# icrdr/3D-UNet-Renal-Anatomy-Extraction

Measured on AMD Instinct MI355X. Metric: train voxels/sec (128^3 patch, bs=2 per GPU), whole job, higher is better.
Workload: dtype bf16; 1 GPU; ResUnet3D(num_pool=4, num_features=32, in=1, out=3) train step (fwd+HybirdLoss+bwd+Adam), 2x1x128^3 per GPU, dropout on; global_batch=2, parallelism=dp1, optimizer=optim.Adam (fused multi-tensor)

## Files before the change

### 3d-unet-renal-anatomy-extraction_amd/_native.py

```python
import ctypes
import os
import threading

import torch

_HERE = os.path.dirname(os.path.abspath(__file__))
LIB_PATH = os.environ.get("RU3D_LIB", os.path.join(_HERE, "libru3d.so"))

F32, BF16, F16 = 0, 1, 2
PREDICT_MAX_BATCH = 16
LABEL_I64, LABEL_U8 = 0, 1
ROLE_CONV_FWD, ROLE_CONV_DGRAD, ROLE_CONVT_FWD, ROLE_CONVT_DGRAD, ROLE_BIAS = 0, 1, 2, 3, 4
LOSS_HYBIRD, LOSS_DICELOSS, LOSS_FOCAL, LOSS_DICE = 0, 1, 2, 3
MAX_CLASSES = 8


class Tensor(ctypes.Structure):
    _fields_ = [("ptr", ctypes.c_void_p), ("n", ctypes.c_int32), ("d", ctypes.c_int32), ("h", ctypes.c_int32),
                ("w", ctypes.c_int32), ("c", ctypes.c_int32), ("ld", ctypes.c_int32), ("cseg", ctypes.c_int32),
                ("seg_stride", ctypes.c_int64)]


class PackItem(ctypes.Structure):
    _fields_ = [("src", ctypes.c_void_p), ("dst", ctypes.c_void_p), ("cout", ctypes.c_int32), ("cin", ctypes.c_int32),
# ... 31 lines not shown
                ("y0", ctypes.c_int32), ("w", ctypes.c_int32), ("h", ctypes.c_int32), ("X", ctypes.c_int32),
                ("Y", ctypes.c_int32), ("Z", ctypes.c_int32), ("C", ctypes.c_int32), ("channel", ctypes.c_int32),
                ("kind", ctypes.c_int32), ("axis", ctypes.c_int32), ("index", ctypes.c_int32),
                ("overlay_mode", ctypes.c_int32 * 2)]


class RenderView(ctypes.Structure):
    _fields_ = [("o", ctypes.c_double * 3), ("du", ctypes.c_double * 3), ("dv", ctypes.c_double * 3),
                ("dw", ctypes.c_double * 3), ("spacing", ctypes.c_double * 3), ("light", ctypes.c_double * 3),
                ("ambient", ctypes.c_double), ("diffuse", ctypes.c_double), ("background", ctypes.c_double * 3),
                ("num_steps", ctypes.c_int32), ("reserved", ctypes.c_int32)]


class DsLevel(ctypes.Structure):
    _fields_ = [("logits", ctypes.c_void_p), ("stride_n", ctypes.c_int64), ("stride_c", ctypes.c_int64),
                ("stride_v", ctypes.c_int64), ("d", ctypes.c_int32), ("h", ctypes.c_int32), ("w", ctypes.c_int32),
                ("shift", ctypes.c_int32)]


DS_MAX_LEVELS = 8
MASK_NE, MASK_EQ, MASK_GT, MASK_GE = 0, 1, 2, 3
TILE_F32, TILE_U8 = 0, 1
OVERLAY_FILL, OVERLAY_OUTLINE = 0, 1
RENDER_MAX_TILES = 256
MORPH_ERODE, MORPH_DILATE = 0, 1
MORPH_MAX_EXTENT, MORPH_MAX_ROWS = 15, 225
CONFUSION_MAX_CLASSES = 32
ORDER_STATS_MAX_RANKS = 8
EDT_MAX_AXIS = 4096
SPATIAL_MAX_YZ = 2560
BOUNDARY_MAX_AXIS = 2048
DEGRADE_MAX_RADIUS = 16
PACK_MAX = 40
_P = ctypes.POINTER(Tensor)
_vp, _i, _i64, _f, _sz, _u64 = (ctypes.c_void_p, ctypes.c_int, ctypes.c_int64, ctypes.c_float, ctypes.c_size_t,
                                ctypes.c_uint64)
_dbl = ctypes.c_double

SIGNATURES = {
    "ru3d_version": (_i, []),
    "ru3d_last_error": (ctypes.c_char_p, []),
    "ru3d_launch_log_begin": (None, []),
    "ru3d_launch_log_end": (ctypes.c_char_p, []),
    "ru3d_packed_weight_bytes": (_sz, [_i, _i, _i, _i, _i, _i]),
    "ru3d_pack_weight": (_i, [_vp, _vp, _i, _i, _i, _i, _i, _i, _vp]),
    "ru3d_pack_weights": (_i, [ctypes.POINTER(PackItem), _i, _i, _vp]),
    "ru3d_unpad_weight_grad": (_i, [_vp, _vp, _i, _i, _i, _i, _i, _vp]),
    "ru3d_conv3d_workspace_bytes": (_sz, [_P, _P, _i, _i, _i]),
    "ru3d_conv3d_fwd": (_i, [_P, _vp, _vp, _P, _P, _i, _i, _i, _i, _vp, _sz, _vp]),
    "ru3d_conv3d_fwd_in_workspace_bytes": (_sz, [_P, _P, _i, _i, _i]),
    "ru3d_conv3d_fwd_in": (_i, [_P, _vp, _vp, _P, _i, _i, _i, _vp, _vp, _vp, _vp, _sz, _f, _vp]),
    "ru3d_conv3d_fwd_in_lrelu_workspace_bytes": (_sz, [_P, _P, _i, _i, _i]),
    "ru3d_conv3d_fwd_in_lrelu": (_i, [_P, _vp, _vp, _P, _i, _i, _i, _vp, _vp, _vp, _P, _P, _f, _vp, _sz, _f, _vp]),
    "ru3d_planar_concat_supported": (_i, [_i, _i, _i, _i, _i, _i, _i]),
    "ru3d_conv3d_dgrad": (_i, [_P, _vp, _P, _P, _i, _i, _i, _vp, _sz, _vp]),
    "ru3d_conv3d_s2_pair_fwd_in_supported": (_i, [_P, _P, _P, _i]),
    "ru3d_conv3d_s2_pair_fwd_in_workspace_bytes": (_sz, [_P, _P, _i]),
    "ru3d_conv3d_s2_pair_fwd_in": (_i, [_P, _vp, _vp, _P, _vp, _vp, _P, _vp, _vp, _vp, _vp, _sz, _f, _i, _vp]),
    "ru3d_conv3d_s1_dgrad_pair_supported": (_i, [_P, _P, _P, _i]),
    "ru3d_conv3d_s1_dgrad_pair": (_i, [_P, _vp, _P, _vp, _P, _i, _vp]),
    "ru3d_conv3d_s2_dgrad_pair_supported": (_i, [_P, _P, _P, _P, _i]),
    "ru3d_conv3d_s2_dgrad_pair": (_i, [_P, _vp, _P, _vp, _P, _P, _i, _vp]),
    "ru3d_conv3d_wgrad_workspace_bytes": (_sz, [_P, _P, _i, _i, _i]),
    "ru3d_conv3d_wgrad": (_i, [_P, _P, _vp, _vp, _sz, _i, _i, _i, _vp]),
    "ru3d_conv3d_wgrad_bias_workspace_bytes": (_sz, [_P, _P, _i, _i, _i]),
    "ru3d_conv3d_wgrad_bias": (_i, [_P, _P, _vp, _vp, _vp, _sz, _i, _i, _i, _vp]),
    "ru3d_conv3d_wgrad_pair_supported": (_i, [_P, _P, _P, _i, _i]),
    "ru3d_conv3d_wgrad_pair_workspace_bytes": (_sz, [_P, _P, _P, _i, _i]),
    "ru3d_conv3d_wgrad_pair": (_i, [_P, _P, _P, _vp, _vp, _vp, _sz, _i, _i, _vp]),
    "ru3d_head_bwd_supported": (_i, [_P, _P, _P, _i]),
    "ru3d_head_bwd_workspace_bytes": (_sz, [_P, _i]),
    "ru3d_head_bwd": (_i, [_P, _P, _vp, _i, _P, _vp, _vp, _vp, _sz, _i, _vp]),
    "ru3d_convtranspose3d_k3s2p1_fwd": (_i, [_P, _vp, _vp, _P, _i, _vp]),
    "ru3d_convtranspose3d_k3s2p1_fwd_in_workspace_bytes": (_sz, [_P, _P, _i]),
    "ru3d_convtranspose3d_k3s2p1_fwd_in": (_i, [_P, _vp, _vp, _P, _vp, _vp, _vp, _sz, _f, _i, _vp]),
    "ru3d_convtranspose3d_k3s2p1_dgrad": (_i, [_P, _vp, _P, _i, _vp]),
    "ru3d_convtranspose3d_k3s2p1_wgrad_workspace_bytes": (_sz, [_P, _P, _i]),
    "ru3d_convtranspose3d_k3s2p1_wgrad": (_i, [_P, _P, _vp, _vp, _sz, _i, _vp]),
    "ru3d_reduce_workspace_bytes": (_sz, [_P]),
    "ru3d_instnorm_stats": (_i, [_P, _vp, _vp, _vp, _vp, _sz, _f, _i, _vp]),
    "ru3d_in_lrelu_fwd": (_i, [_P, _vp, _vp, _P, _P, _f, _i, _vp]),
    "ru3d_skip1x1_in_lrelu_fwd_supported": (_i, [_P, _P, _P, _i]),
    "ru3d_skip1x1_in_lrelu_fwd": (_i, [_P, _vp, _vp, _P, _vp, _vp, _P, _f, _i, _vp]),
    "ru3d_in_lrelu_bwd": (_i, [_P, _P, _P, _vp, _vp, _P, _P, _vp, _sz, _f, _i, _vp, _vp, _i, _vp]),
    "ru3d_in_lrelu_bwd_apply": (_i, [_P, _P, _vp, _vp, _vp, _P, _f, _i, _i, _vp]),
    "ru3d_conv3d_dgrad_in_bwd_workspace_bytes": (_sz, [_P, _P, _i, _i, _i]),
    "ru3d_conv3d_dgrad_in_bwd": (_i, [_P, _vp, _P, _vp, _vp, _P, _P, _i, _i, _f, _i, _vp, _sz, _vp]),
    "ru3d_channel_sum": (_i, [_P, _vp, _vp, _sz, _i, _vp]),
    "ru3d_batchnorm_stats_pool": (_i, [_P, _vp, _vp, _vp, _sz, _i, _vp]),
    "ru3d_batchnorm_stats_finalize": (_i, [_vp, _i, _i, _i, _dbl, _vp, _vp, _vp, _f, _f, _vp, _vp, _vp, _vp, _vp, _vp, _vp]),
    "ru3d_affine_lrelu_fwd": (_i, [_P, _vp, _vp, _P, _P, _f, _i, _vp]),
    "ru3d_batchnorm_bwd_pool": (_i, [_P, _P, _P, _vp, _vp, _P, _vp, _vp, _sz, _f, _i, _vp]),
    "ru3d_batchnorm_bwd_apply": (_i, [_P, _P, _vp, _vp, _vp, _vp, _dbl, _P, _vp, _sz, _i, _i, _vp]),
    "ru3d_dropout3d_scale": (_i, [_vp, _i, _f, _u64, _u64, _vp]),
    "ru3d_dropout3d_scale_dev": (_i, [_vp, _i, _f, _u64, _u64, _vp, _vp]),
    "ru3d_pointwise": (_i, [_i, _P, _P, _P, _P, _P, _f, _i, _vp]),
    "ru3d_copy_channels": (_i, [_P, _P, _i, _vp]),
    "ru3d_add": (_i, [_P, _P, _P, _i, _vp]),
    "ru3d_cast_f32": (_i, [_P, _P, _i, _vp]),
    "ru3d_ncdhw_to_ndhwc": (_i, [_vp, _P, _i, _vp]),
    "ru3d_ndhwc_to_ncdhw": (_i, [_P, _vp, _i, _vp]),
    "ru3d_loss_state_bytes": (_sz, [_i]),
    "ru3d_loss_state_bad_labels_offset": (_sz, []),
    "ru3d_loss_workspace_bytes": (_sz, [_i, _i64, _i]),
    "ru3d_loss_fwd": (_i, [_vp, _i64, _i64, _i64, _vp, _i, _i, _i64, _i, _i, _f, _vp, _f, _f, _f, _vp, _vp, _vp,
                           _sz, _vp]),
    "ru3d_loss_bwd": (_i, [_vp, _i64, _i64, _i64, _vp, _i, _i, _i64, _i, _f, _vp, _vp, _vp, _i, _vp]),
    "ru3d_tversky": (_i, [_vp, _vp, _i64, _f, _f, _f, _vp, _vp, _sz, _vp]),
    "ru3d_predict_accumulate": (_i, [_P, _i, _i, _vp, _vp, _i, _i, _i, _i, _i, _i, _vp]),
    "ru3d_predict_merge": (_i, [_vp, _vp, _i, _i, _i, _i, _i, _i, _i, _i, _i, _i, _i, _vp, _vp]),
    "ru3d_predict_gather": (_i, [_vp, _i, _i, _i, _i, _vp, _i, _P, _vp]),
    "ru3d_predict_accumulate_weighted": (_i, [_P, _i, _i, _i, _vp, _vp, _vp, _vp, _vp, _i, _i, _i, _i, _i, _i, _vp]),
    "ru3d_components_workspace_bytes": (_sz, [_i, _i, _i]),
    "ru3d_label_components": (_i, [_vp, _i, _i, _i, _vp, _vp, _vp, _sz, _vp]),
    "ru3d_component_stats": (_i, [_vp, _i, _i, _i, _i, _vp, _vp, _vp]),
    "ru3d_filter_components_workspace_bytes": (_sz, [_i]),
    "ru3d_filter_components": (_i, [_vp, _i, _i, _i, _i, _vp, _i, _vp, _vp, _vp, _vp, _sz, _vp]),
    "ru3d_region_accumulate": (_i, [_vp, _i, _i, _i, _i, _i, _i, _i, _vp, _vp, _i, _i, _i, _vp]),
    "ru3d_cascade_merge": (_i, [_vp, _vp, _i, _i, _i, _i, _vp, _vp]),
    "ru3d_mask_bytes": (_sz, [_i, _i, _i]),
    "ru3d_mask_pack": (_i, [_vp, _i, _i, _i, _i, _i, _vp, _vp]),
    "ru3d_mask_unpack": (_i, [_vp, _i, _i, _i, _i, _i, _vp, _vp]),
    "ru3d_binary_morph": (_i, [_vp, _vp, _i, _i, _i, _i, ctypes.POINTER(MorphRow), _i, _i, _vp]),
    "ru3d_confusion_counts": (_i, [_vp, _vp, _i64, _i, _vp, _vp]),
    "ru3d_threshold_bbox": (_i, [_vp, _i, _i, _i, _i, _f, _vp, _vp, _vp]),
    "ru3d_masked_sample_workspace_bytes": (_sz, [_i, _i, _i]),
    "ru3d_masked_sample": (_i, [_vp, _i, _i, _i, _i, _i, _vp, _i, _i, _vp, _i64, _vp, _vp, _sz, _vp]),
    "ru3d_order_stats_workspace_bytes": (_sz, []),
    "ru3d_order_stats": (_i, [_vp, _i64, ctypes.POINTER(ctypes.c_int64), _i, _vp, _vp, _sz, _vp]),
    "ru3d_moments_workspace_bytes": (_sz, []),
    "ru3d_moments": (_i, [_vp, _i64, _vp, _vp, _sz, _vp]),
    "ru3d_edt_workspace_bytes": (_sz, [_i, _i, _i]),
    "ru3d_edt_squared": (_i, [_vp, _i, _i, _i, ctypes.POINTER(_dbl), _vp, _vp, _sz, _vp]),
    "ru3d_mask_surface": (_i, [_vp, _vp, _i, _i, _i, _vp]),
    "ru3d_edt_gather_workspace_bytes": (_sz, [_i, _i, _i]),
    "ru3d_edt_gather": (_i, [_vp, _vp, _i, _i, _i, _vp, _i64, _vp, _vp, _sz, _vp]),
    "ru3d_edt_reduce_workspace_bytes": (_sz, [_i64]),
    "ru3d_edt_reduce": (_i, [_vp, _vp, _i64, _dbl, _vp, _vp, _sz, _vp]),
    "ru3d_skeleton_workspace_bytes": (_sz, [_i, _i, _i]),
    "ru3d_skeleton_thin": (_i, [_vp, _i, _i, _i, _i, _vp, _sz, _vp]),
    "ru3d_skeleton_classify": (_i, [_vp, _i, _i, _i, _vp, _vp, _vp, _vp]),
    "ru3d_skeleton_length": (_i, [_vp, _i, _i, _i, ctypes.POINTER(_dbl), _vp, _vp, _sz, _vp]),
    "ru3d_skeleton_overlap": (_i, [_vp, _vp, _i, _i, _i, _vp, _vp]),
    "ru3d_skeleton_radius_stats": (_i, [_vp, _i64, _vp, _vp]),
    "ru3d_cldice_workspace_bytes": (_sz, [_i, _i, _i, _i, _i]),
    "ru3d_cldice_state_bytes": (_sz, []),
    "ru3d_soft_skeleton_fwd": (_i, [_vp, _i, _i, _i, _i, _i, _vp, _vp, _vp, _vp, _vp, _sz, _vp]),
    "ru3d_soft_skeleton_bwd": (_i, [_vp, _i, _i, _i, _i, _i, _vp, _vp, _vp, _vp, _vp, _vp, _sz, _vp]),
    "ru3d_cldice_fwd": (_i, [_vp, _i64, _i64, _i64, _vp, _i, _i, _i, _i, _i, _i, _vp, _i, _i, _vp, _f, _vp, _vp, _vp,
                             _vp, _vp, _vp, _vp, _vp, _sz, _vp]),
    "ru3d_cldice_bwd": (_i, [_vp, _i64, _i64, _i64, _vp, _i, _i, _i, _i, _i, _i, _vp, _i, _i, _vp, _vp, _vp, _vp, _vp,
                             _vp, _vp, _f, _i, _vp, _vp, _sz, _vp]),
    "ru3d_boundary_workspace_bytes": (_sz, [_i, _i, _i, _i]),
    "ru3d_boundary_state_bytes": (_sz, []),
    "ru3d_signed_distance": (_i, [_vp, _i, _i, _i, _i, _i, _i, _vp, _i, _vp, _vp, _vp, _sz, _vp]),
    "ru3d_boundary_fwd": (_i, [_vp, _i64, _i64, _i64, _vp, _i, _i, _i, _i, _i, _i, _vp, _i, _vp, _vp, _vp, _vp, _vp,
                               _sz, _vp]),
    "ru3d_boundary_bwd": (_i, [_vp, _i64, _i64, _i64, _i, _i, _i, _i, _i, _vp, _i, _vp, _vp, _vp, _f, _i, _vp, _vp]),
    "ru3d_ds_state_bytes": (_sz, []),
    "ru3d_ds_state_bad_labels_offset": (_sz, []),
    "ru3d_ds_block_bytes": (_sz, []),
    "ru3d_ds_loss_workspace_bytes": (_sz, [ctypes.POINTER(DsLevel), _i, _i]),
    "ru3d_ds_loss_fwd": (_i, [ctypes.POINTER(DsLevel), _i, _vp, _i, _i, _i, _i, _i, _i, _i, _f, _vp, _f, _f, _f, _vp, _vp,
                              _vp, _vp, _sz, _vp]),
    "ru3d_ds_loss_bwd": (_i, [ctypes.POINTER(DsLevel), ctypes.POINTER(_vp), _i, _vp, _i, _i, _i, _i, _i, _i, _f, _vp, _vp,
                              _vp]),
# ... 217 lines not shown
```

### 3d-unet-renal-anatomy-extraction_amd/_ops.py

```python
import ctypes
import os
import threading
import weakref

import torch

import _native as N
from _native import check, desc, ptr, ref, stream

LRELU_SLOPE = 0.01
IN_EPS = 1e-5


def pack_weight(w, role, dtype, stride=1):
    N.require_device(w, "weight")
    w = w.detach()
    if w.dtype != torch.float32 or not w.is_contiguous():
        w = w.float().contiguous()
    k = w.shape[2]
    if role in (N.ROLE_CONVT_FWD, N.ROLE_CONVT_DGRAD):
        cin, cout = w.shape[0], w.shape[1]
    else:
        cout, cin = w.shape[0], w.shape[1]
    code = N.dtype_code(dtype)
# ... 431 lines not shown
        return None
    dx = N.new_act(2 * n, cin // 2, d, h, w, dy.dtype, dy.device) if planar else N.new_act(n, cin, d, h, w, dy.dtype, dy.device)
    ddy, ddy2, ddx = desc(dy), desc(dy2), desc(N.Split(dx) if planar else dx)
    if not N.lib.ru3d_conv3d_s1_dgrad_pair_supported(ref(ddy), ref(ddy2), ref(ddx), code):
        return None
    check(N.lib.ru3d_conv3d_s1_dgrad_pair(ref(ddy), ptr(pw3), ref(ddy2), ptr(pw1), ref(ddx), code, stream()),
          "conv3d_s1_dgrad_pair")
    return dx


def conv_s2_dgrad_pair(dy, pw3, dy2, pw1, in_shape, res=None):
    n, cin, d, h, w = in_shape
    code = N.dtype_code(dy.dtype)
    if code == N.F32:
        return None
    dx = N.new_act(n, cin, d, h, w, dy.dtype, dy.device)
    ddy, ddy2, ddx = desc(dy), desc(dy2), desc(dx)
    dr = desc(res) if res is not None else None
    if not N.lib.ru3d_conv3d_s2_dgrad_pair_supported(ref(ddy), ref(ddy2), ref(dr), ref(ddx), code):
        return None
    check(N.lib.ru3d_conv3d_s2_dgrad_pair(ref(ddy), ptr(pw3), ref(ddy2), ptr(pw1), ref(dr), ref(ddx), code, stream()),
          "conv3d_s2_dgrad_pair")
    return dx


def convt_dgrad(dy, pw, in_shape):
    n, cin, d, h, w = in_shape
    dx = N.new_act(n, cin, d, h, w, dy.dtype, dy.device)
    ddy, ddx = desc(dy), desc(dx)
    check(N.lib.ru3d_convtranspose3d_k3s2p1_dgrad(ref(ddy), ptr(pw), ref(ddx), N.dtype_code(dy.dtype), stream()),
          "convtranspose3d_dgrad")
    return dx


def convt_wgrad(x, dy, key=None):
    cin, cout = x.shape[1], dy.shape[1]
    dw = _grad_out(key, (cin, cout, 3, 3, 3), x.device)
    dx, ddy = desc(x), desc(dy)
    code = N.dtype_code(x.dtype)
    nbytes = N.lib.ru3d_convtranspose3d_k3s2p1_wgrad_workspace_bytes(ref(dx), ref(ddy), code)
    ws = N.workspace(nbytes, x.device)
    check(N.lib.ru3d_convtranspose3d_k3s2p1_wgrad(ref(dx), ref(ddy), ptr(dw), ptr(ws), ws.numel(), code, stream()),
          "convtranspose3d_wgrad")
    return dw


def in_stats(y, drop_scale=None):
    n, c = y.shape[0], y.shape[1]
    mean = torch.empty(n * c, dtype=torch.float32, device=y.device)
    scale = torch.empty(n * c, dtype=torch.float32, device=y.device)
    dy = desc(y)
    ws = N.workspace(N.lib.ru3d_reduce_workspace_bytes(ref(dy)), y.device)
    check(N.lib.ru3d_instnorm_stats(ref(dy), ptr(drop_scale), ptr(mean), ptr(scale), ptr(ws), ws.numel(), IN_EPS,
                                    N.dtype_code(y.dtype), stream()), "instnorm_stats")
    return mean, scale


def in_lrelu_fwd(y, mean, scale, res=None, out=None):
    if out is None:
        n, c, d, h, w = y.shape
        out = N.new_act(n, c, d, h, w, y.dtype, y.device)
    dy, do = desc(y), desc(out)
    dr = desc(res) if res is not None else None
    check(N.lib.ru3d_in_lrelu_fwd(ref(dy), ptr(mean), ptr(scale), ref(dr), ref(do), LRELU_SLOPE,
                                  N.dtype_code(y.dtype), stream()), "in_lrelu_fwd")
    return out


def skip1x1_in_lrelu_fwd(x, pw, bias, y, mean, scale, out=None):
    code = N.dtype_code(y.dtype)
    if code == N.F32:
        return None
    if out is None:
        n, c, d, h, w = y.shape
        out = N.new_act(n, c, d, h, w, y.dtype, y.device)
    dx, dy, do = desc(x), desc(y), desc(out)
    if not N.lib.ru3d_skip1x1_in_lrelu_fwd_supported(ref(dx), ref(dy), ref(do), code):
        return None
    check(N.lib.ru3d_skip1x1_in_lrelu_fwd(ref(dx), ptr(pw), ptr(_bias(bias)), ref(dy), ptr(mean), ptr(scale), ref(do),
                                          LRELU_SLOPE, code, stream()), "skip1x1_in_lrelu_fwd")
    return out


def in_lrelu_bwd(gout, out, y, mean, scale, want_gpre=False, zero_far=False, want_gpre_sum=False, dy_sum=None):
    n, c, d, h, w = y.shape
    dy = N.new_act(n, c, d, h, w, y.dtype, y.device)
    gpre = N.new_act(n, c, d, h, w, y.dtype, y.device) if want_gpre else None
    dg, do, dyy, ddy = desc(gout), desc(out), desc(y), desc(dy)
    dp = desc(gpre) if want_gpre else None
    ws = N.workspace(N.lib.ru3d_reduce_workspace_bytes(ref(dyy)), y.device)
    gsum = torch.empty(c, dtype=torch.float32, device=y.device) if (want_gpre and want_gpre_sum) else None
    check(N.lib.ru3d_in_lrelu_bwd(ref(dg), ref(do), ref(dyy), ptr(mean), ptr(scale), ref(ddy), ref(dp), ptr(ws),
                                  ws.numel(), LRELU_SLOPE, 1 if zero_far else 0, ptr(gsum), ptr(dy_sum),
                                  N.dtype_code(y.dtype), stream()), "in_lrelu_bwd")
    if want_gpre_sum:
        return dy, gpre, gsum
    return dy, gpre


_BN_SYNC = [None, 1]


def set_bn_sync(group=None, enable=True):
    import torch.distributed as dist
    if enable and dist.is_available() and dist.is_initialized() and dist.get_world_size(group) > 1:
        _BN_SYNC[0], _BN_SYNC[1] = (group if group is not None else dist.group.WORLD), dist.get_world_size(group)
    else:
        _BN_SYNC[0], _BN_SYNC[1] = None, 1


def _bn_allreduce(pooled):
    if _BN_SYNC[0] is not None:
        import torch.distributed as dist
        dist.all_reduce(pooled, group=_BN_SYNC[0])
    return pooled


def bn_train_stats(y, drop_scale, norm, c_real):
    n, c = y.shape[0], y.shape[1]
    dev = y.device
    dy = desc(y)
    pooled = torch.empty(2 * c, dtype=torch.float64, device=dev)
    ws = N.workspace(N.lib.ru3d_reduce_workspace_bytes(ref(dy)), dev)
    check(N.lib.ru3d_batchnorm_stats_pool(ref(dy), ptr(drop_scale), ptr(pooled), ptr(ws), ws.numel(),
                                          N.dtype_code(y.dtype), stream()), "batchnorm_stats_pool")
    _bn_allreduce(pooled)
    count = float(n * y.shape[2] * y.shape[3] * y.shape[4]) * _BN_SYNC[1]
    track = norm.track_running_stats and norm.running_mean is not None
    momentum = 0.0
    if track:
        norm.num_batches_tracked.add_(1)
        momentum = (1.0 / float(norm.num_batches_tracked)) if norm.momentum is None else float(norm.momentum)
    out = torch.empty(4, n * c, dtype=torch.float32, device=dev)
    gamma = norm.weight.detach() if norm.weight is not None else None
    beta = norm.bias.detach() if norm.bias is not None else None
    for t in (gamma, beta, norm.running_mean if track else None, norm.running_var if track else None):
        if t is not None and (t.dtype != torch.float32 or not t.is_contiguous() or t.device != dev):
            raise N.Ru3dError("BatchNorm3d: parameters / running statistics must be contiguous fp32 on %s" % dev)
    check(N.lib.ru3d_batchnorm_stats_finalize(ptr(pooled), n, c, c_real, count, ptr(drop_scale), ptr(gamma), ptr(beta),
                                              float(norm.eps), momentum, ptr(norm.running_mean if track else None),
                                              ptr(norm.running_var if track else None), ptr(out[0]), ptr(out[1]),
                                              ptr(out[2]), ptr(out[3]), stream()), "batchnorm_stats_finalize")
    return out[0], out[1], out[2], out[3], count


def affine_lrelu_fwd(y, scale, shift, res=None, out=None):
    if out is None:
        n, c, d, h, w = y.shape
        out = N.new_act(n, c, d, h, w, y.dtype, y.device)
    dy, do = desc(y), desc(out)
    dr = desc(res) if res is not None else None
    check(N.lib.ru3d_affine_lrelu_fwd(ref(dy), ptr(scale), ptr(shift), ref(dr), ref(do), LRELU_SLOPE,
                                      N.dtype_code(y.dtype), stream()), "affine_lrelu_fwd")
    return out


def bn_lrelu_bwd(gout, out, y, a, b, fscale, count, zero_far=False):
    n, c, d, h, w = y.shape
    dev = y.device
    dy = N.new_act(n, c, d, h, w, y.dtype, dev)
    gpre = N.new_act(n, c, d, h, w, y.dtype, dev)
    dg, do, dyy, ddy, dp = desc(gout), desc(out), desc(y), desc(dy), desc(gpre)
    pooled = torch.empty(2 * c, dtype=torch.float64, device=dev)
    ws = N.workspace(N.lib.ru3d_reduce_workspace_bytes(ref(dyy)), dev)
    code = N.dtype_code(y.dtype)
    check(N.lib.ru3d_batchnorm_bwd_pool(ref(dg), ref(do), ref(dyy), ptr(a), ptr(b), ref(dp), ptr(pooled), ptr(ws),
# ... 215 lines not shown
    def skip_view(self, n, c, d, h, w, dtype, device):
        self.planar = False
        self.buf = N.new_act(n, self.up_channels + c, d, h, w, dtype, device)
        return self.buf[:, self.up_channels:]

    def planar_view(self, n, c, d, h, w, dtype, device):
        if (c != self.up_channels or dtype == torch.float32 or not self.dec_channels
                or not N.lib.ru3d_planar_concat_supported(n, d, h, w, c, self.dec_channels, N.dtype_code(dtype))):
            return None
        self.planar = True
        self.buf = N.new_act(2 * n, c, d, h, w, dtype, device)
        return self.buf[n:]


def _f32_view(pack, count):
    return pack[:4 * count].view(torch.float32)


class ConvFn(torch.autograd.Function):

    @staticmethod
    def forward(ctx, x, weight, bias, stride, storage_dtype, out_dtype, pad_in=False, pad_out=False):
        xin = as_input(x, storage_dtype)
        k = weight.shape[2]
        cout, cin = weight.shape[0], weight.shape[1]
        cin_seg = seg_of(cin, xin.shape[1]) if pad_in else 0
        cout_seg = cout if pad_out else 0
        if not pad_in and xin.shape[1] != cin:
            raise N.Ru3dError("conv: input has %d channels, weight expects %d" % (xin.shape[1], cin))
        cout_p = padded_dim(cout, cout_seg)
        specs = [(weight, N.ROLE_CONV_FWD, stride, cout_seg, cin_seg)]
        if ctx.needs_input_grad[0]:
            specs.append((weight, N.ROLE_CONV_DGRAD, stride, cout_seg, cin_seg))
        if cout_seg and bias is not None:
            specs.append((bias, N.ROLE_BIAS, 1, cout_seg, 0))
        packs = pack_weights(specs, storage_dtype)
        b = _f32_view(packs[-1], cout_p) if (cout_seg and bias is not None) else bias
        y = conv_fwd(xin, packs[0], b, cout_p, k, stride, out_dtype=out_dtype)
        ctx.save_for_backward(xin, packs[1] if ctx.needs_input_grad[0] else None)
        ctx.dims = (cout, cin, cout_seg, cin_seg)
        ctx.stride, ctx.k, ctx.has_bias = stride, k, bias is not None
        ctx.storage_dtype = storage_dtype
        ctx.in_dtype = x.dtype
        ctx.wkey = weight.data_ptr() if not (cout_seg or cin_seg) else None
        ctx.weight_ref = weight if (k == 1 and cout <= 4) else None
        return y

    @staticmethod
    def backward(ctx, gy):
        xin, pwd = ctx.saved_tensors
        sd = ctx.storage_dtype
        cout, cin, cout_seg, cin_seg = ctx.dims
        if (ctx.k == 1 and ctx.stride == 1 and cout <= 4 and not cout_seg and all(ctx.needs_input_grad[:2])
                and ctx.weight_ref is not None):
            fused = head_bwd(xin, gy, ctx.weight_ref, ctx.has_bias and ctx.needs_input_grad[2],
                             key=None if cin_seg else ctx.wkey)
            if fused is not None:
                gx, gw, gb = fused
                if gx.dtype != ctx.in_dtype:
                    gx = gx.to(ctx.in_dtype)
                return gx, gw, gb, None, None, None, None, None
        gy = as_grad(gy, sd)
        gx = gw = gb = None
        with _OnSide(gy.device):
            if ctx.needs_input_grad[1] and ctx.has_bias and ctx.needs_input_grad[2] and not (cout_seg or cin_seg) \
                    and sd != torch.float32:
                gw, gb = conv_wgrad_bias(xin, gy, ctx.k, ctx.stride, key=ctx.wkey)
            elif ctx.needs_input_grad[1]:
                gw = unpad_wgrad(conv_wgrad(xin, gy, ctx.k, ctx.stride, key=ctx.wkey), cout, cin, cout_seg, cin_seg)
            if gb is None and ctx.has_bias and ctx.needs_input_grad[2]:
                gb = channel_sum(gy)[:cout]
        if ctx.needs_input_grad[0]:
            gx = conv_dgrad(gy, pwd, tuple(xin.shape), ctx.k, ctx.stride)
            if gx.dtype != ctx.in_dtype:
                gx = gx.to(ctx.in_dtype)
        _join(gy.device, gw, gb)
        return gx, gw, gb, None, None, None, None, None


class ResBlockFn(torch.autograd.Function):

    @staticmethod
    def forward(ctx, x, w1, b1, w2, b2, ws, bs, stride, drop_scale, pad=0, checkpoint=False, in_link=None,
                out_link=None, planar=False):
        sd = x.dtype
        x = N.to_ndhwc(x)
        xt = x
        if planar:
            x = N.Split(x)
        cout, cin = w1.shape[0], w1.shape[1]
        cin_seg = seg_of(cin, x.shape[1], int(pad)) if pad else 0
        cout_seg = cout if pad else 0
        if not pad and x.shape[1] != cin:
            raise N.Ru3dError("ResBlock: input has %d channels, conv1 expects %d" % (x.shape[1], cin))
        cout_p = padded_dim(cout, cout_seg)
        train = any(ctx.needs_input_grad)
        need_gx = ctx.needs_input_grad[0]
        specs = [(w1, N.ROLE_CONV_FWD, stride, cout_seg, cin_seg), (w2, N.ROLE_CONV_FWD, 1, cout_seg, cout_seg)]
        if ws is not None:
            specs.append((ws, N.ROLE_CONV_FWD, stride, cout_seg, cin_seg))
        nfwd = len(specs)
        if train:
            specs.append((w2, N.ROLE_CONV_DGRAD, 1, cout_seg, cout_seg))
            if need_gx:
                specs.append((w1, N.ROLE_CONV_DGRAD, stride, cout_seg, cin_seg))
                if ws is not None:
                    specs.append((ws, N.ROLE_CONV_DGRAD, stride, cout_seg, cin_seg))
        nw = len(specs)
        if cout_seg:
            specs += [(b, N.ROLE_BIAS, 1, cout_seg, 0) for b in (b1, b2, bs) if b is not None]
        packs = pack_weights(specs, sd)
        if cout_seg:
            it = iter(packs[nw:])
            b1, b2, bs = [(_f32_view(next(it), cout_p) if b is not None else None) for b in (b1, b2, bs)]
        pw1, pw2 = packs[0], packs[1]
        fused = conv_s2_pair_fwd_in(x, pw1, b1, packs[2], bs, cout_p, drop_scale) if (ws is not None and stride == 2) else None
        if fused is not None:
            y1, mean1, scale1, skip = fused
            a1 = in_lrelu_fwd(y1, mean1, scale1)
        else:
            y1, mean1, scale1, a1 = conv_fwd_in_act(x, pw1, b1, cout_p, 3, stride, drop_scale)
        n_, _, d_, h_, w_ = a1.shape
        zout = None
        if out_link is not None and cout_p * a1.element_size() >= 128:
            zout = out_link.skip_view(n_, cout_p, d_, h_, w_, sd, x.device)
        elif out_link is not None:
            zout = out_link.planar_view(n_, cout_p, d_, h_, w_, sd, x.device)
        z = None
        tail = (fused is None and ws is not None and stride == 1 and out_link is None and sd != torch.float32
                and (x.shape[1], cout_p) in ((64, 32), (128, 64)) and n_ * d_ * h_ * w_ >= 65536)
        if tail:
            y2, mean2, scale2 = conv_fwd_in(a1, pw2, b2, cout_p, 3, 1)
            z = skip1x1_in_lrelu_fwd(x, packs[2], bs, y2, mean2, scale2)
            if z is None:
                z = in_lrelu_fwd(y2, mean2, scale2, res=conv_fwd(x, packs[2], bs, cout_p, 1, stride), out=zout)
        else:
            if fused is not None:
                pass
            elif ws is not None:
                skip = conv_fwd(x, packs[2], bs, cout_p, 1, stride)
            else:
                skip = x
            y2, mean2, scale2, z = conv_fwd_in_act(a1, pw2, b2, cout_p, 3, 1, res=skip, out=zout)
        bwd = packs[nfwd:nw] + [None] * 3
        if checkpoint and train:
            ctx.save_for_backward(xt, None, None, None, z, mean1, scale1, mean2, scale2, bwd[0], bwd[1], bwd[2],
                                  pw1, pw2, b1, b2)
        else:
            ctx.save_for_backward(xt, y1, a1, y2, z, mean1, scale1, mean2, scale2, bwd[0], bwd[1], bwd[2],
                                  None, None, None, None)
        ctx.planar = bool(planar)
        ctx.dims = (cout, cin, cout_seg, cin_seg)
        ctx.stride = stride
        plain = not (cout_seg or cin_seg)
        ctx.wkeys = (w1.data_ptr() if plain else None, w2.data_ptr() if plain else None,
                     ws.data_ptr() if (plain and ws is not None) else None)
        ctx.has_skip_conv = ws is not None
        ctx.in_link = in_link if (in_link is not None and ws is not None) else None
        if in_link is not None:
            in_link.fused_grad = ctx.in_link is not None and need_gx
        return z

    @staticmethod
    def backward(ctx, gz):
        (x, y1, a1, y2, z, mean1, scale1, mean2, scale2, pw2d, pw1d, pwsd, pw1, pw2, b1, b2) = ctx.saved_tensors
        cout, cin, cout_seg, cin_seg = ctx.dims
        cout_p = padded_dim(cout, cout_seg)
        sd = x.dtype
        dev = x.device
        stride = ctx.stride
        gz = as_grad(gz, sd)
        if ctx.planar:
            x = N.Split(x)
        if y1 is None:
            y1 = conv_fwd(x, pw1, b1, cout_p, 3, stride)
            a1 = in_lrelu_fwd(y1, mean1, scale1)
            y2 = conv_fwd(a1, pw2, b2, cout_p, 3, 1)
        dy2, gpre, gbs_sum = in_lrelu_bwd(gz, z, y2, mean2, scale2, want_gpre=True, want_gpre_sum=True)
        del y2
        return ResBlockFn._backward_tail(ctx, x, a1, y1, dy2, gpre, gbs_sum, mean1, scale1, pw2d, pw1d, pwsd)

    @staticmethod
    def _backward_tail(ctx, x, a1, y1, dy2, gpre, gbs_sum, mean1, scale1, pw2d, pw1d, pwsd):
        cout, cin, cout_seg, cin_seg = ctx.dims
        dev = x.device
        stride = ctx.stride
        gws = gbs = None
        nvox = dy2.shape[0] * dy2.shape[2] * dy2.shape[3] * dy2.shape[4]
        xk = x.t if ctx.planar else x
        pair_later = ctx.has_skip_conv and _wgrad_pair_ok(x, gpre, stride)
        with _OnSide(dev, nvox, (a1, dy2, xk, gpre)):
            gw2 = unpad_wgrad(conv_wgrad(a1, dy2, 3, 1, key=ctx.wkeys[1]), cout, cout, cout_seg, cout_seg)
            if ctx.has_skip_conv:
                if not pair_later:
                    gws = unpad_wgrad(conv_wgrad(x, gpre, 1, stride, key=ctx.wkeys[2]), cout, cin, cout_seg, cin_seg)
                gbs = gbs_sum[:cout]
        gb2 = None
        dy1 = conv_dgrad_in_bwd(dy2, pw2d, a1, mean1, scale1)
        del dy2, a1, y1
        with _OnSide(dev, nvox, (xk, dy1, gpre)):
            both = conv_wgrad_pair(x, dy1, gpre, stride, key=ctx.wkeys[0], key2=ctx.wkeys[2]) if pair_later else None
            if both is not None:
                gw1 = unpad_wgrad(both[0], cout, cin, cout_seg, cin_seg)
                gws = unpad_wgrad(both[1], cout, cin, cout_seg, cin_seg)
            else:
                gw1 = unpad_wgrad(conv_wgrad(x, dy1, 3, stride, key=ctx.wkeys[0]), cout, cin, cout_seg, cin_seg)
                if pair_later:
                    gws = unpad_wgrad(conv_wgrad(x, gpre, 1, stride, key=ctx.wkeys[2]), cout, cin, cout_seg, cin_seg)
        gb1 = None
        gx = None
        need_gx = ctx.needs_input_grad[0]
        if ctx.has_skip_conv:
            if need_gx:
                parked = None
                if ctx.in_link is not None:
                    parked, ctx.in_link.grad = ctx.in_link.grad, None
                if stride == 2:
                    gx = conv_s2_dgrad_pair(dy1, pw1d, gpre, pwsd, tuple(x.shape), res=parked)
                elif parked is None:
                    gx = conv_s1_dgrad_pair(dy1, pw1d, gpre, pwsd, tuple(x.shape), planar=ctx.planar)
                if gx is None and ctx.planar:
                    raise N.Ru3dError("ResBlock: the split concat input has no fused input-gradient kernel for this shape")
                if gx is None:
                    gx0 = conv_dgrad(gpre, pwsd, tuple(x.shape), 1, stride, res=parked)
                    gx = conv_dgrad(dy1, pw1d, tuple(x.shape), 3, stride, res=gx0)
        elif need_gx:
            gx = conv_dgrad(dy1, pw1d, tuple(x.shape), 3, stride, res=gpre)
        _join(dev, gw1, gw2, gws, gbs)
        return gx, gw1, gb1, gw2, gb2, gws, gbs, None, None, None, None, None, None, None


class UpFn(torch.autograd.Function):

    @staticmethod
    def forward(ctx, x, wt, bt, skip, pad=False, link=None):
        sd = x.dtype
        x = N.to_ndhwc(x)
        cin, cout = wt.shape[0], wt.shape[1]
        cin_seg = seg_of(cin, x.shape[1]) if pad else 0
        cout_seg = cout if pad else 0
        if not pad and x.shape[1] != cin:
            raise N.Ru3dError("ConvTrans3D: input has %d channels, weight expects %d" % (x.shape[1], cin))
        cout_p = padded_dim(cout, cout_seg)
        specs = [(wt, N.ROLE_CONVT_FWD, 2, cout_seg, cin_seg)]
        if ctx.needs_input_grad[0]:
            specs.append((wt, N.ROLE_CONVT_DGRAD, 2, cout_seg, cin_seg))
        if cout_seg and bt is not None:
            specs.append((bt, N.ROLE_BIAS, 1, cout_seg, 0))
        packs = pack_weights(specs, sd)
        btp = _f32_view(packs[-1], cout_p) if (cout_seg and bt is not None) else bt
        y, mean, scale = convt_fwd_in(x, packs[0], btp, cout_p)
        n, _, d, h, w = y.shape
        if skip is not None:
            skip = as_grad(skip, sd)
            cs = skip.shape[1]
            if tuple(skip.shape[2:]) != (d, h, w) or skip.shape[0] != n:
                raise N.Ru3dError("UpConcat: skip %s does not match up-sampled %s" % (tuple(skip.shape), tuple(y.shape)))
            planar = (link is not None and link.planar and link.buf is not None and link.up_channels == cout_p == cs
                      and tuple(link.buf.shape) == (2 * n, cs, d, h, w) and link.buf.dtype == sd
                      and skip.data_ptr() == link.buf[n:].data_ptr())
            in_place = (not planar and link is not None and not link.planar and link.buf is not None
                        and link.up_channels == cout_p
                        and tuple(link.buf.shape) == (n, cout_p + cs, d, h, w) and link.buf.dtype == sd
# ... 237 lines not shown
```

### 3d-unet-renal-anatomy-extraction_amd/csrc/api.hip

```cpp
#include "common.h"
#include "conv.h"
#include <string>

#ifndef RU3D_STORAGE_F16

static thread_local std::string g_last_error;

int ru3d_fail(int code, const char* fmt, ...) {
    char buf[512];
    va_list ap;
    va_start(ap, fmt);
    vsnprintf(buf, sizeof(buf), fmt, ap);
    va_end(ap);
    g_last_error = buf;
    return code;
}

static thread_local std::string g_launch_log;
static thread_local bool g_launch_log_armed = false;

int ru3d_check_launch(const char* what) {
    if (g_launch_log_armed) {
        if (!g_launch_log.empty()) g_launch_log += ';';
        g_launch_log += what;
// ... 331 lines not shown
    if (!mode || dtype != RU3D_BF16 || n <= 0 || d <= 0 || h <= 0 || w <= 0 || cseg != 32 || cout != 32) return 0;
    const int64_t V = (int64_t)d * h * w;
    if (((int64_t)n * V + V) * cseg * 2 >= (1ll << 31)) return 0;
    SlidePlan sp;
    if (!slide64_conv_plan(n, d, h, w, 2 * cseg, cout, &sp)) return 0;
    ConvGeom gd;
    gd.N = n; gd.Di = gd.Do = d; gd.Hi = gd.Ho = h; gd.Wi = gd.Wo = w; gd.Cin = cout; gd.Cout = 2 * cseg;
    gd.ldx = cout; gd.ldy = cseg; gd.CoutPad = 2 * cseg; gd.ldr = 0; gd.k = 3; gd.stride = 1; gd.pad = 1;
    gd.transposed = 0; gd.zero_far = 0; gd.flip = 1;
    static const int pair_mode = getenv("RU3D_DGRAD_PAIR") ? atoi(getenv("RU3D_DGRAD_PAIR")) : 1;
    if (!pair_mode || !mfma_conv_eligible(gd.Cin, gd.Cout, 3, dtype, dtype) || !mfma_conv_can_fuse_partner(gd)) return 0;
    WgradGeom gw;
    gw.N = n; gw.Di = gw.Do = d; gw.Hi = gw.Ho = h; gw.Wi = gw.Wo = w; gw.Cin = 2 * cseg; gw.Cout = cout;
    gw.ldx = cseg; gw.lddy = cout; gw.k = 3; gw.taps = 27; gw.stride = 1; gw.pad = 1;
    gw.s_o = (int64_t)gw.Cin * 27; gw.s_i = 27; gw.chunk_len = 0;
    WgradSlidePlan wp;
    if (!wgrad_slide_plan(gw, &wp)) return 0;
    static const int skip_mode = getenv("RU3D_FUSED_SKIP") ? atoi(getenv("RU3D_FUSED_SKIP")) : 1;
    if (!skip_mode || (V % 16) != 0 || V * n < 65536) return 0;
    return 1;
}

extern "C" int ru3d_conv3d_dgrad(const ru3d_tensor* dy, const void* w_packed, const ru3d_tensor* res,
                                 const ru3d_tensor* dx, int k, int stride, int dtype, void* ws, size_t ws_bytes,
                                 void* stream) {
    RU3D_FWD_F16(dtype, ru3d_conv3d_dgrad_f16(dy, w_packed, res, dx, k, stride, dtype, ws, ws_bytes, stream));
    Ru3dDeviceGuard dev_guard(stream);
    RU3D_REQUIRE(tensor_ok(dy) && tensor_ok(dx) && w_packed, "conv3d_dgrad: bad tensor/weight");
    RU3D_REQUIRE((k == 1 || k == 3) && (stride == 1 || stride == 2), "conv3d_dgrad: k=%d stride=%d unsupported", k, stride);
    RU3D_REQUIRE(dtype_ok(dtype), "conv3d_dgrad: bad dtype");
    RU3D_REQUIRE(dx->n == dy->n && dy->d == conv_out(dx->d, k, stride) && dy->h == conv_out(dx->h, k, stride) &&
                     dy->w == conv_out(dx->w, k, stride),
                 "conv3d_dgrad: dy extents (%d,%d,%d) do not match dx (%d,%d,%d) k=%d s=%d", dy->d, dy->h, dy->w,
                 dx->d, dx->h, dx->w, k, stride);
    RU3D_REQUIRE(res_ok(res, dx), "conv3d_dgrad: residual shape mismatch");
    if (stride == 1)
        return run_conv(dy, w_packed, nullptr, res, dx, k, 1, 0, 1, 0, dtype, dtype, as_stream(stream), ws, ws_bytes);
    return run_conv(dy, w_packed, nullptr, res, dx, k, stride, 1, 0, 0, dtype, dtype, as_stream(stream));
}

static ConvGeom dgrad_s1_geom(const ru3d_tensor* dy, const ru3d_tensor* da, int k);
extern "C" int ru3d_conv3d_s1_dgrad_pair_supported(const ru3d_tensor* dy, const ru3d_tensor* dy2, const ru3d_tensor* dx, int dtype) {
    RU3D_FWD_F16(dtype, ru3d_conv3d_s1_dgrad_pair_supported_f16(dy, dy2, dx, dtype));
    static const int mode = getenv("RU3D_DGRAD_PAIR") ? atoi(getenv("RU3D_DGRAD_PAIR")) : 1;
    if (!mode || dtype != RU3D_BF16 || !tensor_ok(dy) || !tensor_ok(dy2) || !tensor_ok_split(dx)) return 0;
    if (dx->cseg && (dx->cseg != 32 || dx->c != 64)) return 0;
    if (dy2->n != dy->n || dy2->d != dy->d || dy2->h != dy->h || dy2->w != dy->w || dy2->c != dy->c) return 0;
    if (dx->n != dy->n || dx->d != dy->d || dx->h != dy->h || dx->w != dy->w) return 0;
    if ((dy->ld % 8) || (dy2->ld % 8) || (dx->ld % 8)) return 0;
    if ((((uintptr_t)dy->ptr) | ((uintptr_t)dy2->ptr) | ((uintptr_t)dx->ptr)) % 16) return 0;
    if ((int64_t)dy->d * dy->h * dy->w * dy->ld >= (1ll << 30)) return 0;
    const ConvGeom g = dgrad_s1_geom(dy, dx, 3);
    return (mfma_conv_eligible(g.Cin, g.Cout, 3, dtype, dtype) && mfma_conv_can_fuse_partner(g)) ? 1 : 0;
}

extern "C" int ru3d_conv3d_s1_dgrad_pair(const ru3d_tensor* dy, const void* w3_packed, const ru3d_tensor* dy2,
                                         const void* w1_packed, const ru3d_tensor* dx, int dtype, void* stream) {
    RU3D_FWD_F16(dtype, ru3d_conv3d_s1_dgrad_pair_f16(dy, w3_packed, dy2, w1_packed, dx, dtype, stream));
    Ru3dDeviceGuard dev_guard(stream);
    RU3D_REQUIRE(w3_packed && w1_packed, "conv3d_s1_dgrad_pair: null weight");
    RU3D_REQUIRE(ru3d_conv3d_s1_dgrad_pair_supported(dy, dy2, dx, dtype),
                 "conv3d_s1_dgrad_pair: shapes have no fused kernel (ask ru3d_conv3d_s1_dgrad_pair_supported first)");
    const ConvGeom g = dgrad_s1_geom(dy, dx, 3);
    return conv_mfma_launch(dy->ptr, w3_packed, nullptr, nullptr, dx->ptr, g, as_stream(stream), nullptr, nullptr, 0, nullptr, 0,
                            0.f, dy2->ptr, dy2->ld, w1_packed);
}

extern "C" int ru3d_skip1x1_in_lrelu_fwd_supported(const ru3d_tensor* x, const ru3d_tensor* y, const ru3d_tensor* out, int dtype) {
    RU3D_FWD_F16(dtype, ru3d_skip1x1_in_lrelu_fwd_supported_f16(x, y, out, dtype));
    return skip1x1_fused_eligible(x, y, out, dtype) ? 1 : 0;
}

extern "C" int ru3d_skip1x1_in_lrelu_fwd(const ru3d_tensor* x, const void* w_packed, const float* bias, const ru3d_tensor* y,
                                         const float* mean, const float* scale, const ru3d_tensor* out, float slope, int dtype,
                                         void* stream) {
    RU3D_FWD_F16(dtype, ru3d_skip1x1_in_lrelu_fwd_f16(x, w_packed, bias, y, mean, scale, out, slope, dtype, stream));
    Ru3dDeviceGuard dev_guard(stream);
    RU3D_REQUIRE(w_packed && mean && scale, "skip1x1_in_lrelu_fwd: null argument");
    RU3D_REQUIRE(skip1x1_fused_eligible(x, y, out, dtype),
                 "skip1x1_in_lrelu_fwd: shapes have no fused kernel (ask ru3d_skip1x1_in_lrelu_fwd_supported first)");
    return skip1x1_fused_launch(x, w_packed, bias, y, mean, scale, out, slope, as_stream(stream));
}

extern "C" int ru3d_conv3d_s2_pair_fwd_in_supported(const ru3d_tensor* x, const ru3d_tensor* y3, const ru3d_tensor* y1, int dtype) {
    RU3D_FWD_F16(dtype, ru3d_conv3d_s2_pair_fwd_in_supported_f16(x, y3, y1, dtype));
    if (dtype != RU3D_BF16 || !tensor_ok(x) || !tensor_ok(y3) || !tensor_ok(y1)) return 0;
    if (y3->n != x->n || y3->d != conv_out(x->d, 3, 2) || y3->h != conv_out(x->h, 3, 2) || y3->w != conv_out(x->w, 3, 2)) return 0;
    if (y1->n != y3->n || y1->d != y3->d || y1->h != y3->h || y1->w != y3->w || y1->c != y3->c) return 0;
    if ((y1->ld % 4) || (int64_t)y1->d * y1->h * y1->w * y1->ld >= (1ll << 30)) return 0;
    if ((((uintptr_t)x->ptr) % 16) || ((((uintptr_t)y3->ptr) | ((uintptr_t)y1->ptr)) % 8)) return 0;
    return conv_s2_tile_eligible(fwd_geom(x, y3, 3, 2)) ? 1 : 0;
}

extern "C" size_t ru3d_conv3d_s2_pair_fwd_in_workspace_bytes(const ru3d_tensor* x, const ru3d_tensor* y3, int dtype) {
    RU3D_FWD_F16(dtype, ru3d_conv3d_s2_pair_fwd_in_workspace_bytes_f16(x, y3, dtype));
    if (!tensor_ok(x) || !tensor_ok(y3)) return 0;
    return conv_s2_tile_slab_bytes(fwd_geom(x, y3, 3, 2));
}

extern "C" int ru3d_conv3d_s2_pair_fwd_in(const ru3d_tensor* x, const void* w3_packed, const float* b3, const ru3d_tensor* y3,
                                          const void* w1_packed, const float* b1, const ru3d_tensor* y1,
                                          const float* drop_scale, float* mean, float* scale, void* ws, size_t ws_bytes,
                                          float eps, int dtype, void* stream) {
    RU3D_FWD_F16(dtype, ru3d_conv3d_s2_pair_fwd_in_f16(x, w3_packed, b3, y3, w1_packed, b1, y1, drop_scale, mean, scale, ws, ws_bytes, eps, dtype, stream));
    Ru3dDeviceGuard dev_guard(stream);
    RU3D_REQUIRE(w3_packed && w1_packed && mean && scale && ws, "conv3d_s2_pair_fwd_in: null argument");
    RU3D_REQUIRE(ru3d_conv3d_s2_pair_fwd_in_supported(x, y3, y1, dtype),
                 "conv3d_s2_pair_fwd_in: shapes have no fused kernel (ask ru3d_conv3d_s2_pair_fwd_in_supported first)");
    const ConvGeom g = fwd_geom(x, y3, 3, 2);
    const size_t slab = conv_s2_tile_slab_bytes(g);
    RU3D_REQUIRE(ws_bytes >= slab, "conv3d_s2_pair_fwd_in: workspace too small");
    int rc = conv_s2_tile_launch(x->ptr, w3_packed, b3, y3->ptr, g, (float*)ws, w1_packed, b1, y1->ptr, y1->ld, as_stream(stream));
    if (rc) return rc;
    int gx, cb;
    if (conv_s2_tile_slab_geom(g, &gx, &cb)) return ru3d_fail(-1, "conv3d_s2_pair_fwd_in: no slab geometry");
    return stats_slab_finalize_launch((const float*)ws, gx, cb, g.N, g.Cout, 1.0 / ((double)g.Do * g.Ho * g.Wo), drop_scale, eps,
                                      mean, scale, as_stream(stream));
}

static ConvGeom s2_dgrad_geom(const ru3d_tensor* dy, const ru3d_tensor* res, const ru3d_tensor* dx) {
    ConvGeom g;
    g.N = dy->n;
    g.Di = dy->d; g.Hi = dy->h; g.Wi = dy->w; g.Cin = dy->c; g.ldx = dy->ld;
    g.Do = dx->d; g.Ho = dx->h; g.Wo = dx->w; g.Cout = dx->c; g.ldy = dx->ld;
    g.CoutPad = generic_cout_pad(dx->c);
    g.ldr = res ? res->ld : 0;
    g.k = 3; g.stride = 2; g.pad = 1;
    g.transposed = 1; g.zero_far = 0; g.flip = 0;
    return g;
}

extern "C" int ru3d_conv3d_s2_dgrad_pair_supported(const ru3d_tensor* dy, const ru3d_tensor* dy2, const ru3d_tensor* res,
                                                   const ru3d_tensor* dx, int dtype) {
    RU3D_FWD_F16(dtype, ru3d_conv3d_s2_dgrad_pair_supported_f16(dy, dy2, res, dx, dtype));
    if (dtype != RU3D_BF16 || !tensor_ok(dy) || !tensor_ok(dy2) || !tensor_ok(dx) || !res_ok(res, dx)) return 0;
    if (dy2->n != dy->n || dy2->d != dy->d || dy2->h != dy->h || dy2->w != dy->w || dy2->c != dy->c) return 0;
    if (dx->n != dy->n || dy->d != conv_out(dx->d, 3, 2) || dy->h != conv_out(dx->h, 3, 2) || dy->w != conv_out(dx->w, 3, 2))
        return 0;
    if ((dy2->ld % 8) || (int64_t)dy2->d * dy2->h * dy2->w * dy2->ld >= (1ll << 30)) return 0;
    if ((((uintptr_t)dy->ptr) | ((uintptr_t)dy2->ptr) | ((uintptr_t)dx->ptr) | (res ? (uintptr_t)res->ptr : 0)) % 16) return 0;
    return convt_s2_tile_eligible(s2_dgrad_geom(dy, res, dx)) ? 1 : 0;
}

extern "C" int ru3d_conv3d_s2_dgrad_pair(const ru3d_tensor* dy, const void* w3_packed, const ru3d_tensor* dy2,
                                         const void* w1_packed, const ru3d_tensor* res, const ru3d_tensor* dx, int dtype,
                                         void* stream) {
    RU3D_FWD_F16(dtype, ru3d_conv3d_s2_dgrad_pair_f16(dy, w3_packed, dy2, w1_packed, res, dx, dtype, stream));
    Ru3dDeviceGuard dev_guard(stream);
    RU3D_REQUIRE(w3_packed && w1_packed, "conv3d_s2_dgrad_pair: null weight");
    RU3D_REQUIRE(ru3d_conv3d_s2_dgrad_pair_supported(dy, dy2, res, dx, dtype),
                 "conv3d_s2_dgrad_pair: shapes have no fused kernel (ask ru3d_conv3d_s2_dgrad_pair_supported first)");
    const ConvGeom g = s2_dgrad_geom(dy, res, dx);
    return convt_s2_tile_launch(dy->ptr, w3_packed, nullptr, res ? res->ptr : nullptr, dx->ptr, g, nullptr, dy2->ptr,
                                dy2->ld, w1_packed, as_stream(stream));
}

static ConvGeom dgrad_s1_geom(const ru3d_tensor* dy, const ru3d_tensor* da, int k) {
    ConvGeom g = fwd_geom(dy, da, k, 1);
    g.flip = 1;
    return g;
}

static bool dgrad_in_bwd_fused(const ru3d_tensor* dy, const ru3d_tensor* da, int k, int stride, int dtype) {
    static const int mode = getenv("RU3D_DGRAD_IN_FUSE") ? atoi(getenv("RU3D_DGRAD_IN_FUSE")) : 1;
    if (!mode || k != 3 || stride != 1 || dtype == RU3D_F32) return false;
    const ConvGeom g = dgrad_s1_geom(dy, da, k);
// ... 307 lines not shown
```

### 3d-unet-renal-anatomy-extraction_amd/csrc/conv.h

```cpp
#pragma once
#include "common.h"

namespace RU3D_NS {

struct ConvGeom {
    int N;
    int Di, Hi, Wi, Cin, ldx;
    int Do, Ho, Wo, Cout, ldy;
    int CoutPad;
    int ldr;
    int k, stride, pad;
    int transposed;
    int zero_far;
    int flip;
    int x_cseg = 0, y_cseg = 0;
    int64_t x_segstride = 0, y_segstride = 0;
};

struct WgradGeom {
    int N;
    int Di, Hi, Wi, Cin, ldx;
    int Do, Ho, Wo, Cout, lddy;
    int k, taps, stride, pad;
    int64_t s_o, s_i;
// ... 15 lines not shown
};
int pack_batch_launch(const PackBatch& b, int dtype, hipStream_t st);

struct PackPair {
    const float* src;
    void* dst_a;
    void* dst_b;
    int adim, bdim, taps;
    int a_real, a_pad, b_real, b_pad;
    int64_t s_a;
};
struct PackPairBatch {
    int count;
    PackPair item[RU3D_PACK_MAX];
};
int pack_pair_launch(const PackPairBatch& b, hipStream_t st);
int unpad_weight_launch(const float* src, float* dst, int cout, int cin, int taps, int co_real, int co_pad, int ci_real,
                        int ci_pad, int cin_p, hipStream_t st);

int generic_cot(int cout);
int generic_cout_pad(int cout);
int conv_generic_launch(const void* x, const void* w, const float* bias, const void* res, void* y,
                        const ConvGeom& g, int dtype, int y_dtype, hipStream_t st);
int pack_generic_launch(const float* src, void* dst, int cin, int cout, int taps, int64_t s_o, int64_t s_i,
                        int flip, int dtype, hipStream_t st);
size_t wgrad_generic_ws_bytes(const WgradGeom& g);
int wgrad_reduce_launch(const float* part, float* dw, int chunks, int taps, int cin, int cout, int64_t s_o, int64_t s_i,
                        hipStream_t st);
int wgrad_generic_launch(const void* x, const void* dy, float* dw, void* ws, size_t ws_bytes, WgradGeom g, int dtype,
                         hipStream_t st);

bool mfma_conv_eligible(int cin, int cout, int k, int dtype, int y_dtype);
bool mfma_conv_geometry_ok(const ConvGeom& g);
size_t mfma_packed_bytes(int cin, int cout, int taps);
int pack_mfma_launch(const float* src, void* dst, int cin, int cout, int taps, int64_t s_o, int64_t s_i, int flip,
                     hipStream_t st);
int conv_mfma_launch(const void* x, const void* w, const float* bias, const void* res, void* y, const ConvGeom& g,
                     hipStream_t st, float* stat_slab = nullptr, void* ws = nullptr, size_t ws_bytes = 0,
                     const void* bst_act = nullptr, int bst_ld = 0, float slope = 0.f, const void* x2 = nullptr,
                     int ldx2 = 0, const void* w2 = nullptr, int* defer_ks = nullptr);
bool mfma_conv_can_fuse_partner(const ConvGeom& g);
size_t conv_mfma_ws_bytes(const ConvGeom& g);
bool mfma_conv_can_fuse_stats(const ConvGeom& g);
size_t mfma_conv_stats_slab_bytes(const ConvGeom& g);
int mfma_conv_stats_finalize(const ConvGeom& g, const float* slab, const float* drop, float eps, float* mean,
                             float* scale, hipStream_t st);
int stats_slab_finalize_launch(const float* slab, int gx, int cb, int N, int C, double invV, const float* drop, float eps,
                               float* mean, float* scale, hipStream_t st);
bool mfma_conv_can_fuse_bwd_sums(const ConvGeom& g);
int mfma_conv_bwd_sums_finalize(const ConvGeom& g, const float* slab, float* m12, hipStream_t st);
bool mfma_wgrad_eligible(const WgradGeom& g, int dtype);
size_t wgrad_mfma_ws_bytes(const WgradGeom& g);
int wgrad_mfma_launch(const void* x, const void* dy, float* dw, void* ws, size_t ws_bytes, WgradGeom g,
                      hipStream_t st);

struct SlidePlan {
    int dsplit, DL, tiles_h, tiles_w, units, grid, ny;
};
bool slide_conv_plan(int N, int D, int H, int W, int Cin, int Cout, SlidePlan* out);
int conv_slide_launch(const void* x, const void* w, const float* bias, const void* res, void* y, const ConvGeom& g,
                      float* stat_slab, hipStream_t st, const void* bst_act = nullptr, int bst_ld = 0, float slope = 0.f,
                      const void* x2 = nullptr, int ldx2 = 0, const void* w2 = nullptr);

bool slide64_conv_plan(int N, int D, int H, int W, int Cin, int Cout, SlidePlan* out);
int conv_ws_slices(int N, int D, int H, int W, int Cin, int Cout);
int conv_ws_launch(const void* x, const void* w, float* part, int N, int D, int H, int W, int Cin, int Cout, int ldx,
                   int flip, int slices, hipStream_t st);
int conv_slide64_launch(const void* x, const void* w, const float* bias, const void* res, void* y, const ConvGeom& g,
                        float* stat_slab, hipStream_t st, const void* bst_act = nullptr, int bst_ld = 0, float slope = 0.f);

bool convt_s2_tile_eligible(const ConvGeom& g);
size_t convt_s2_tile_slab_bytes(const ConvGeom& g);
int convt_s2_tile_slab_geom(const ConvGeom& g, int* gx, int* cb);
int convt_s2_tile_launch(const void* x, const void* w, const float* bias, const void* res, void* y, const ConvGeom& g,
                         float* stat_slab, const void* x2, int ldx2, const void* w2, hipStream_t st);

bool conv_s2_tile_eligible(const ConvGeom& g);
size_t conv_s2_tile_slab_bytes(const ConvGeom& g);
int conv_s2_tile_slab_geom(const ConvGeom& g, int* gx, int* cb);
int conv_s2_tile_launch(const void* x, const void* w, const float* bias, void* y, const ConvGeom& g, float* stat_slab,
                        const void* w2, const float* bias2, void* y2, int ldy2, hipStream_t st);

bool skip1x1_fused_eligible(const ru3d_tensor* x, const ru3d_tensor* y2, const ru3d_tensor* out, int dtype);
int skip1x1_fused_launch(const ru3d_tensor* x, const void* w, const float* bias, const ru3d_tensor* y2, const float* mean,
                         const float* scale, const ru3d_tensor* out, float slope, hipStream_t st);

int in_small_mode(const ru3d_tensor* y, bool all_samples, const ru3d_tensor* a = nullptr, const ru3d_tensor* b = nullptr,
                  const ru3d_tensor* c = nullptr, const ru3d_tensor* d = nullptr);
size_t in_small_ws_bytes(const ru3d_tensor* y);
int in_small_fwd_launch(const ru3d_tensor* y, const float* part, int ksplit, const float* bias, const float* drop,
                        float* mean, float* scale, const ru3d_tensor* res, const ru3d_tensor* out, void* ws, float eps,
                        float slope, hipStream_t st);
int in_small_bwd_launch(const ru3d_tensor* gout, const float* part, int ksplit, const ru3d_tensor* outp,
                        const ru3d_tensor* y, const float* mean, const float* scale, const ru3d_tensor* dy,
                        const ru3d_tensor* gpre, void* ws, float slope, int zero_far, float* gpre_sum, hipStream_t st);

struct WgradSlidePlan {
    int dsplit, DL, tiles_h, tiles_w, units, G, pairs;
};
bool wgrad_slide_plan(const WgradGeom& g, WgradSlidePlan* out);
size_t wgrad_slide_ws_bytes(const WgradGeom& g);
int wgrad_slide_launch(const void* x, const void* dy, float* dw, void* ws, const WgradGeom& g, hipStream_t st);
size_t wgrad_slide_pair_ws_bytes(const WgradGeom& g);
int wgrad_slide_pair_launch(const void* x, const void* dy, const void* dy2, int lddy2, float* dw, float* dw2, void* ws,
                            const WgradGeom& g, hipStream_t st);

bool wgrad_s2_eligible(const WgradGeom& g);
size_t wgrad_s2_ws_bytes(const WgradGeom& g);
int wgrad_s2_launch(const void* x, const void* dy, float* dw, void* ws, const WgradGeom& g, hipStream_t st);
bool wgrad_s2_pair_eligible(const WgradGeom& g);
size_t wgrad_s2_pair_ws_bytes(const WgradGeom& g);
int wgrad_s2_pair_launch(const void* x, const void* dy, const void* dy2, int lddy2, float* dw, float* dw2, void* ws,
                         const WgradGeom& g, hipStream_t st);

bool stem_fwd_eligible(const ConvGeom& g, int dtype, int y_dtype, const void* res);
int stem_fwd_launch(const void* x, const void* w, const float* bias, void* y, const ConvGeom& g, int dtype,
                    hipStream_t st);
bool head_fwd_eligible(const ConvGeom& g, int dtype, const void* res);
int head_fwd_launch(const void* x, const void* w, const float* bias, void* y, const ConvGeom& g, int dtype,
                    int y_dtype, hipStream_t st);
bool head_dgrad_eligible(const ConvGeom& g, int dtype, int y_dtype, const void* res);
int head_dgrad_launch(const void* dy, const void* w, void* dx, const ConvGeom& g, int dtype, hipStream_t st);
bool stem_wgrad_eligible(const WgradGeom& g);
size_t stem_wgrad_ws_bytes(const WgradGeom& g);
int stem_wgrad_launch(const void* x, const void* dy, float* dw, void* ws, size_t ws_bytes, const WgradGeom& g,
                      int dtype, hipStream_t st, float* db = nullptr);
bool stem_wgrad_gives_bias(const WgradGeom& g, int dtype);
bool head_bwd_eligible(int Cin, int Cout, int dtype);
size_t head_bwd_ws_bytes(int64_t P, int Cin);
int head_bwd_launch(const void* a, int lda, const float* dlog, int ldd, const float* w, int cin_real, int Cin, int Cout,
                    void* dx, int lddx, float* dw, float* db, void* ws, int64_t P, hipStream_t st);
bool head_wgrad_eligible(const WgradGeom& g, int dtype);
size_t head_wgrad_ws_bytes(const WgradGeom& g);
int head_wgrad_launch(const void* x, const void* dy, float* dw, void* ws, size_t ws_bytes, const WgradGeom& g,
                      int dtype, hipStream_t st);

}
using namespace RU3D_NS;
```

### 3d-unet-renal-anatomy-extraction_amd/csrc/f16_names.h

```cpp
#pragma once
#define RU3D_F16_APIS(X) \
    X(ru3d_packed_weight_bytes) \
    X(ru3d_pack_weight) \
    X(ru3d_pack_weights) \
    X(ru3d_conv3d_workspace_bytes) \
    X(ru3d_conv3d_fwd) \
    X(ru3d_conv3d_fwd_in_workspace_bytes) \
    X(ru3d_conv3d_fwd_in) \
    X(ru3d_conv3d_fwd_in_lrelu) \
    X(ru3d_planar_concat_supported) \
    X(ru3d_conv3d_dgrad) \
    X(ru3d_conv3d_s2_pair_fwd_in_supported) \
    X(ru3d_conv3d_s2_pair_fwd_in_workspace_bytes) \
    X(ru3d_conv3d_s2_pair_fwd_in) \
    X(ru3d_conv3d_s1_dgrad_pair_supported) \
    X(ru3d_conv3d_s1_dgrad_pair) \
    X(ru3d_conv3d_s2_dgrad_pair_supported) \
    X(ru3d_conv3d_s2_dgrad_pair) \
    X(ru3d_convtranspose3d_k3s2p1_fwd_in_workspace_bytes) \
    X(ru3d_convtranspose3d_k3s2p1_fwd_in) \
    X(ru3d_conv3d_dgrad_in_bwd_workspace_bytes) \
    X(ru3d_conv3d_dgrad_in_bwd) \
    X(ru3d_in_lrelu_bwd_apply) \
    X(ru3d_conv3d_wgrad_workspace_bytes) \
    X(ru3d_conv3d_wgrad) \
    X(ru3d_conv3d_wgrad_bias_workspace_bytes) \
    X(ru3d_conv3d_wgrad_bias) \
    X(ru3d_conv3d_wgrad_pair_supported) \
    X(ru3d_conv3d_wgrad_pair_workspace_bytes) \
    X(ru3d_conv3d_wgrad_pair) \
    X(ru3d_head_bwd_supported) \
    X(ru3d_head_bwd_workspace_bytes) \
    X(ru3d_head_bwd) \
    X(ru3d_convtranspose3d_k3s2p1_fwd) \
    X(ru3d_convtranspose3d_k3s2p1_dgrad) \
    X(ru3d_convtranspose3d_k3s2p1_wgrad_workspace_bytes) \
    X(ru3d_convtranspose3d_k3s2p1_wgrad) \
    X(ru3d_instnorm_stats) \
    X(ru3d_in_lrelu_fwd) \
    X(ru3d_skip1x1_in_lrelu_fwd_supported) \
    X(ru3d_skip1x1_in_lrelu_fwd) \
    X(ru3d_in_lrelu_bwd) \
    X(ru3d_channel_sum) \
    X(ru3d_copy_channels) \
    X(ru3d_add) \
    X(ru3d_cast_f32) \
    X(ru3d_ncdhw_to_ndhwc) \
    X(ru3d_ndhwc_to_ncdhw) \
    X(ru3d_pointwise) \
    X(ru3d_batchnorm_stats_pool) \
    X(ru3d_affine_lrelu_fwd) \
    X(ru3d_batchnorm_bwd_pool) \
    X(ru3d_batchnorm_bwd_apply)

#ifdef RU3D_STORAGE_F16
#define ru3d_packed_weight_bytes ru3d_packed_weight_bytes_f16
#define ru3d_pack_weight ru3d_pack_weight_f16
#define ru3d_pack_weights ru3d_pack_weights_f16
#define ru3d_conv3d_workspace_bytes ru3d_conv3d_workspace_bytes_f16
#define ru3d_conv3d_fwd ru3d_conv3d_fwd_f16
#define ru3d_conv3d_fwd_in_workspace_bytes ru3d_conv3d_fwd_in_workspace_bytes_f16
#define ru3d_conv3d_fwd_in ru3d_conv3d_fwd_in_f16
#define ru3d_conv3d_fwd_in_lrelu ru3d_conv3d_fwd_in_lrelu_f16
#define ru3d_planar_concat_supported ru3d_planar_concat_supported_f16
#define ru3d_conv3d_dgrad ru3d_conv3d_dgrad_f16
#define ru3d_conv3d_s2_pair_fwd_in_supported ru3d_conv3d_s2_pair_fwd_in_supported_f16
#define ru3d_conv3d_s2_pair_fwd_in_workspace_bytes ru3d_conv3d_s2_pair_fwd_in_workspace_bytes_f16
#define ru3d_conv3d_s2_pair_fwd_in ru3d_conv3d_s2_pair_fwd_in_f16
#define ru3d_conv3d_s1_dgrad_pair_supported ru3d_conv3d_s1_dgrad_pair_supported_f16
#define ru3d_conv3d_s1_dgrad_pair ru3d_conv3d_s1_dgrad_pair_f16
#define ru3d_conv3d_s2_dgrad_pair_supported ru3d_conv3d_s2_dgrad_pair_supported_f16
#define ru3d_conv3d_s2_dgrad_pair ru3d_conv3d_s2_dgrad_pair_f16
#define ru3d_convtranspose3d_k3s2p1_fwd_in_workspace_bytes ru3d_convtranspose3d_k3s2p1_fwd_in_workspace_bytes_f16
#define ru3d_convtranspose3d_k3s2p1_fwd_in ru3d_convtranspose3d_k3s2p1_fwd_in_f16
#define ru3d_conv3d_dgrad_in_bwd_workspace_bytes ru3d_conv3d_dgrad_in_bwd_workspace_bytes_f16
#define ru3d_conv3d_dgrad_in_bwd ru3d_conv3d_dgrad_in_bwd_f16
#define ru3d_in_lrelu_bwd_apply ru3d_in_lrelu_bwd_apply_f16
#define ru3d_conv3d_wgrad_workspace_bytes ru3d_conv3d_wgrad_workspace_bytes_f16
#define ru3d_conv3d_wgrad ru3d_conv3d_wgrad_f16
#define ru3d_conv3d_wgrad_bias_workspace_bytes ru3d_conv3d_wgrad_bias_workspace_bytes_f16
#define ru3d_conv3d_wgrad_bias ru3d_conv3d_wgrad_bias_f16
#define ru3d_conv3d_wgrad_pair_supported ru3d_conv3d_wgrad_pair_supported_f16
#define ru3d_conv3d_wgrad_pair_workspace_bytes ru3d_conv3d_wgrad_pair_workspace_bytes_f16
#define ru3d_conv3d_wgrad_pair ru3d_conv3d_wgrad_pair_f16
#define ru3d_head_bwd_supported ru3d_head_bwd_supported_f16
#define ru3d_head_bwd_workspace_bytes ru3d_head_bwd_workspace_bytes_f16
#define ru3d_head_bwd ru3d_head_bwd_f16
#define ru3d_convtranspose3d_k3s2p1_fwd ru3d_convtranspose3d_k3s2p1_fwd_f16
#define ru3d_convtranspose3d_k3s2p1_dgrad ru3d_convtranspose3d_k3s2p1_dgrad_f16
#define ru3d_convtranspose3d_k3s2p1_wgrad_workspace_bytes ru3d_convtranspose3d_k3s2p1_wgrad_workspace_bytes_f16
#define ru3d_convtranspose3d_k3s2p1_wgrad ru3d_convtranspose3d_k3s2p1_wgrad_f16
#define ru3d_instnorm_stats ru3d_instnorm_stats_f16
#define ru3d_in_lrelu_fwd ru3d_in_lrelu_fwd_f16
#define ru3d_skip1x1_in_lrelu_fwd_supported ru3d_skip1x1_in_lrelu_fwd_supported_f16
#define ru3d_skip1x1_in_lrelu_fwd ru3d_skip1x1_in_lrelu_fwd_f16
#define ru3d_in_lrelu_bwd ru3d_in_lrelu_bwd_f16
#define ru3d_channel_sum ru3d_channel_sum_f16
#define ru3d_copy_channels ru3d_copy_channels_f16
#define ru3d_add ru3d_add_f16
#define ru3d_cast_f32 ru3d_cast_f32_f16
#define ru3d_ncdhw_to_ndhwc ru3d_ncdhw_to_ndhwc_f16
#define ru3d_ndhwc_to_ncdhw ru3d_ndhwc_to_ncdhw_f16
#define ru3d_pointwise ru3d_pointwise_f16
#define ru3d_batchnorm_stats_pool ru3d_batchnorm_stats_pool_f16
#define ru3d_affine_lrelu_fwd ru3d_affine_lrelu_fwd_f16
#define ru3d_batchnorm_bwd_pool ru3d_batchnorm_bwd_pool_f16
#define ru3d_batchnorm_bwd_apply ru3d_batchnorm_bwd_apply_f16
#endif
```

### 3d-unet-renal-anatomy-extraction_amd/csrc/fused_skip.hip

```cpp
#include "common.h"
#include "conv.h"

#include <type_traits>

namespace RU3D_NS {
namespace {

#ifdef RU3D_STORAGE_F16
#define RU3D_MFMA_16X16X32 __builtin_amdgcn_mfma_f32_16x16x32_f16
#else
#define RU3D_MFMA_16X16X32 __builtin_amdgcn_mfma_f32_16x16x32_bf16
#endif

template <int I, int N, typename F>
__device__ __forceinline__ void static_for(F&& f) {
    if constexpr (I < N) {
        f(std::integral_constant<int, I>{});
        static_for<I + 1, N>(f);
    }
}

typedef float f32x8 __attribute__((ext_vector_type(8)));

struct SkipArgs {
    const bf16* x;
    const bf16x8* w;
    const float* bias;
    const bf16* y2;
    const float* mean;
    const float* scale;
    bf16* out;
    int N;
    int64_t V;
    int ldx, ldy, ldo;
    int cout;
    float slope;
    int x_cseg;
    int64_t x_segstride;
};

template <int CIN, int NPB>
__global__ __launch_bounds__(256) void skip1x1_in_lrelu_fwd_kernel(SkipArgs a) {
    constexpr int KS = CIN / 32;
    const int lane = threadIdx.x & 63;
    const int p = lane & 15, g4 = lane >> 4;
    const int NTT = a.cout / 32;

    bf16x8 wreg[KS * NPB * 2];
    static_for<0, KS * NPB * 2>([&](auto ic) {
        constexpr int i = decltype(ic)::value;
        constexpr int ks = i / (NPB * 2), pb = (i / 2) % NPB, t = i & 1;
        const int co = pb * 32 + 8 * (p >> 2) + 4 * t + (p & 3);
        const int ci8 = ks * 4 + g4;
        wreg[i] = a.w[((ci8 >> 1) * NTT + (co >> 5)) * 64 + (co & 31) + 32 * (ci8 & 1)];
    });
    float bias8[NPB][8];
#pragma unroll
    for (int pb = 0; pb < NPB; pb++)
#pragma unroll
        for (int i = 0; i < 8; i++) bias8[pb][i] = a.bias ? a.bias[pb * 32 + 8 * g4 + i] : 0.f;

    const int64_t groups_per_sample = a.V / 16;
    const int64_t total = groups_per_sample * a.N;
    const int64_t wave_id = (int64_t)blockIdx.x * 4 + (threadIdx.x >> 6);
    const int64_t nwaves = (int64_t)gridDim.x * 4;
    int cur_n = -1;
    float mu[NPB][8], sc[NPB][8];
    for (int64_t gi = wave_id; gi < total; gi += nwaves) {
        const int n = (int)(gi / groups_per_sample);
        if (n != cur_n) {
            cur_n = n;
#pragma unroll
            for (int pb = 0; pb < NPB; pb++)
#pragma unroll
                for (int i = 0; i < 8; i++) {
                    mu[pb][i] = a.mean[n * a.cout + pb * 32 + 8 * g4 + i];
                    sc[pb][i] = a.scale[n * a.cout + pb * 32 + 8 * g4 + i];
                }
        }
        const int64_t vox = gi * 16 + p;
        bf16x8 xb[KS];
        static_for<0, KS>([&](auto kc) {
            constexpr int ks = decltype(kc)::value;
            const bf16* xp = a.x_cseg ? a.x + (int64_t)((ks * 32) / a.x_cseg) * a.x_segstride + (ks * 32) % a.x_cseg
                                      : a.x + ks * 32;
            xb[ks] = *reinterpret_cast<const bf16x8*>(xp + vox * a.ldx + g4 * 8);
        });
        bf16x8 yv[NPB];
#pragma unroll
        for (int pb = 0; pb < NPB; pb++) yv[pb] = *reinterpret_cast<const bf16x8*>(a.y2 + vox * a.ldy + pb * 32 + 8 * g4);
        f32x4 acc[NPB][2];
#pragma unroll
        for (int pb = 0; pb < NPB; pb++) {
            acc[pb][0] = f32x4{bias8[pb][0], bias8[pb][1], bias8[pb][2], bias8[pb][3]};
            acc[pb][1] = f32x4{bias8[pb][4], bias8[pb][5], bias8[pb][6], bias8[pb][7]};
        }
        static_for<0, KS>([&](auto kc) {
            constexpr int ks = decltype(kc)::value;
            static_for<0, NPB * 2>([&](auto tc) {
                constexpr int j = decltype(tc)::value;
                acc[j >> 1][j & 1] = RU3D_MFMA_16X16X32(wreg[ks * NPB * 2 + j], xb[ks], acc[j >> 1][j & 1], 0, 0, 0);
            });
        });
#pragma unroll
        for (int pb = 0; pb < NPB; pb++) {
            f32x4 a0 = acc[pb][0], a1 = acc[pb][1];
            asm("s_nop 7\n\ts_nop 4" : "+v"(a0), "+v"(a1));
            const f32x8 s = {a0[0], a0[1], a0[2], a0[3], a1[0], a1[1], a1[2], a1[3]};
            const bf16x8 sk = __builtin_convertvector(s, bf16x8);
            f32x8 o;
#pragma unroll
            for (int i = 0; i < 8; i++) {
                const float t = ((float)yv[pb][i] - mu[pb][i]) * sc[pb][i] + (float)sk[i];
                o[i] = t > 0.f ? t : t * a.slope;
            }
            *reinterpret_cast<bf16x8*>(a.out + vox * a.ldo + pb * 32 + 8 * g4) = __builtin_convertvector(o, bf16x8);
        }
    }
}

}

bool skip1x1_fused_eligible(const ru3d_tensor* x, const ru3d_tensor* y2, const ru3d_tensor* out, int dtype) {
    static const int mode = getenv("RU3D_FUSED_SKIP") ? atoi(getenv("RU3D_FUSED_SKIP")) : 1;
    if (!mode || dtype != RU3D_BF16) return false;
    if (!tensor_ok_split(x) || !tensor_ok(y2) || !tensor_ok(out)) return false;
    if (x->cseg && (x->cseg % 32)) return false;
    if (x->n != y2->n || x->d != y2->d || x->h != y2->h || x->w != y2->w) return false;
    if (out->n != y2->n || out->d != y2->d || out->h != y2->h || out->w != y2->w || out->c != y2->c) return false;
    if (!((x->c == 64 && y2->c == 32) || (x->c == 128 && y2->c == 64))) return false;
    if ((x->ld % 8) || (y2->ld % 8) || (out->ld % 8)) return false;
    if ((((uintptr_t)x->ptr) | ((uintptr_t)y2->ptr) | ((uintptr_t)out->ptr)) % 16) return false;
    const int64_t V = (int64_t)x->d * x->h * x->w;
    return (V % 16) == 0 && V * x->n >= 65536;
}

int skip1x1_fused_launch(const ru3d_tensor* x, const void* w, const float* bias, const ru3d_tensor* y2, const float* mean,
                         const float* scale, const ru3d_tensor* out, float slope, hipStream_t st) {
    SkipArgs a;
    a.x = (const bf16*)x->ptr; a.w = (const bf16x8*)w; a.bias = bias; a.y2 = (const bf16*)y2->ptr;
    a.mean = mean; a.scale = scale; a.out = (bf16*)out->ptr;
    a.N = x->n;
    a.V = (int64_t)x->d * x->h * x->w;
    a.ldx = x->ld; a.ldy = y2->ld; a.ldo = out->ld;
    a.cout = y2->c;
    a.slope = slope;
    a.x_cseg = x->cseg; a.x_segstride = x->seg_stride;
    const int64_t groups = a.V / 16 * a.N;
    int64_t blocks = (groups + 3) / 4;
    const int64_t cap = 256 * 8;
    if (blocks > cap) blocks = cap;
    if (x->c == 64) hipLaunchKernelGGL((skip1x1_in_lrelu_fwd_kernel<64, 1>), dim3((unsigned)blocks), dim3(256), 0, st, a);
    else hipLaunchKernelGGL((skip1x1_in_lrelu_fwd_kernel<128, 2>), dim3((unsigned)blocks), dim3(256), 0, st, a);
    return ru3d_check_launch("skip1x1_in_lrelu_fwd");
}

}
```

### 3d-unet-renal-anatomy-extraction_amd/csrc/norm.hip

```cpp
#include "common.h"
#include "conv.h"
#include <initializer_list>

namespace RU3D_NS {

struct ChanLoop {
    int V;
    int G;
    int Gb;
    int vpb;
    int span;
    int chunks;
};

static ChanLoop make_chanloop(int64_t V, int C, int vec, int max_iters, int N = 1) {
    ChanLoop cl;
    cl.V = (int)V;
    cl.G = C / vec;
    cl.Gb = cl.G < 256 ? cl.G : 256;
    cl.vpb = 256 / cl.Gb;
    const int64_t gz = (cl.G + cl.Gb - 1) / cl.Gb;
    int64_t iters = (V * N * gz + (int64_t)cl.vpb * 2048 - 1) / ((int64_t)cl.vpb * 2048);
    if (iters < 4) iters = 4;
    if (iters > max_iters) iters = max_iters;
// ... 486 lines not shown
    RU3D_REQUIRE(mean && scale, "in_lrelu_fwd: null stats");
    RU3D_REQUIRE((int64_t)y->d * y->h * y->w < (1ll << 31), "in_lrelu_fwd: sample too large");
    if (dtype == RU3D_F32) return in_fwd_impl<float>(y, mean, scale, res, out, slope, as_stream(stream));
    if (dtype == RU3D_BF16) return in_fwd_impl<bf16>(y, mean, scale, res, out, slope, as_stream(stream));
    return ru3d_fail(-1, "in_lrelu_fwd: bad dtype %d", dtype);
}

template <typename T>
static int in_bwd_impl(const ru3d_tensor* gout, const ru3d_tensor* out, const ru3d_tensor* y, const float* mean,
                       const float* scale, const ru3d_tensor* dy, const ru3d_tensor* gpre, void* ws, float slope,
                       int zero_far, float* gpre_sum, float* dy_sum, hipStream_t st) {
    const int64_t V = (int64_t)y->d * y->h * y->w;
    const int vec = pick_vec<T>(y->c, {gout, out, y, dy, gpre});
    ChanLoop cl = make_chanloop(V, y->c, vec, 64, y->n);
    dim3 grid(cl.chunks, y->n, (cl.G + cl.Gb - 1) / cl.Gb);
    double* part = (double*)ws;
    float* m12 = (float*)((char*)ws + (size_t)y->n * cl.chunks * y->c * 2 * sizeof(double));
#define CALL(TT, VV)                                                                                                  \
    if (gpre)                                                                                                         \
        hipLaunchKernelGGL((reduce2_kernel<TT, VV, 4>), grid, dim3(256), 0, st, (const TT*)gout->ptr, gout->ld,       \
                           (const TT*)out->ptr, out->ld, (const TT*)y->ptr, y->ld, mean, scale, slope, part, cl,      \
                           y->c, (TT*)gpre->ptr, gpre->ld);                                                           \
    else                                                                                                              \
        hipLaunchKernelGGL((reduce2_kernel<TT, VV, 3>), grid, dim3(256), 0, st, (const TT*)gout->ptr, gout->ld,       \
                           (const TT*)out->ptr, out->ld, (const TT*)0, 0, mean, scale, slope, part, cl, y->c)
    DISPATCH_VEC(T, vec, CALL)
#undef CALL
    int rc = ru3d_check_launch("in_lrelu_bwd_reduce");
    if (rc) return rc;
    hipLaunchKernelGGL(bwd_finalize_kernel, dim3((y->c + FIN_CX - 1) / FIN_CX), dim3(256), 0, st, (const double*)part,
                       cl.chunks, y->c, y->n, 1.0 / (double)V, m12, (double)V, gpre_sum);
    rc = ru3d_check_launch("in_lrelu_bwd_finalize");
    if (rc) return rc;
    ChanLoop ca = make_chanloop(V, y->c, vec, 16, y->n);
    dim3 grida(ca.chunks, y->n, (ca.G + ca.Gb - 1) / ca.Gb);
    double* dpart =
        dy_sum ? (double*)((char*)m12 + (((size_t)y->n * y->c * 2 * sizeof(float) + 255) / 256) * 256) : nullptr;
#define CALL(TT, VV)                                                                                                  \
    if (gpre)                                                                                                         \
        hipLaunchKernelGGL((in_lrelu_bwd_kernel<TT, VV, true, true>), grida, dim3(256), 0, st, (const TT*)gout->ptr,  \
                           gout->ld, (const TT*)out->ptr, out->ld, (const TT*)y->ptr, y->ld, mean, scale,            \
                           (const float*)m12, (TT*)dy->ptr, dy->ld, (TT*)gpre->ptr, gpre->ld, slope, zero_far, y->d,  \
                           y->h, y->w, ca, y->c, (const float*)nullptr, (const float*)nullptr, dpart);               \
    else                                                                                                              \
        hipLaunchKernelGGL((in_lrelu_bwd_kernel<TT, VV, false>), grida, dim3(256), 0, st, (const TT*)gout->ptr,       \
                           gout->ld, (const TT*)out->ptr, out->ld, (const TT*)y->ptr, y->ld, mean, scale,            \
                           (const float*)m12, (TT*)dy->ptr, dy->ld, (TT*)0, 0, slope, zero_far, y->d, y->h, y->w, ca, \
                           y->c, (const float*)nullptr, (const float*)nullptr, dpart)
    DISPATCH_VEC(T, vec, CALL)
#undef CALL
    rc = ru3d_check_launch("in_lrelu_bwd_apply");
    if (rc || !dy_sum) return rc;
    hipLaunchKernelGGL(chansum_finalize_kernel, dim3((y->c + FIN_CX - 1) / FIN_CX), dim3(256), 0, st,
                       (const double*)dpart, ca.chunks, y->c, y->n, dy_sum);
    return ru3d_check_launch("in_lrelu_bwd_dysum_finalize");
}

extern "C" int ru3d_in_lrelu_bwd(const ru3d_tensor* gout, const ru3d_tensor* out, const ru3d_tensor* y,
                                 const float* mean, const float* scale, const ru3d_tensor* dy,
                                 const ru3d_tensor* gpre, void* ws, size_t ws_bytes, float slope, int zero_far,
                                 float* gpre_sum, float* dy_sum, int dtype, void* stream) {
    RU3D_FWD_F16(dtype, ru3d_in_lrelu_bwd_f16(gout, out, y, mean, scale, dy, gpre, ws, ws_bytes, slope, zero_far, gpre_sum, dy_sum, dtype, stream));
    Ru3dDeviceGuard dev_guard(stream);
    RU3D_REQUIRE(!gpre_sum || gpre, "in_lrelu_bwd: gpre_sum needs the residual form (gpre != NULL)");
    RU3D_REQUIRE(tensor_ok(gout) && tensor_ok(out) && tensor_ok(y) && tensor_ok(dy), "in_lrelu_bwd: bad tensor");
    RU3D_REQUIRE(same_shape(y, gout) && same_shape(y, out) && same_shape(y, dy), "in_lrelu_bwd: shape mismatch");
    RU3D_REQUIRE(!gpre || (tensor_ok(gpre) && same_shape(y, gpre)), "in_lrelu_bwd: bad gpre");
    RU3D_REQUIRE(mean && scale && ws, "in_lrelu_bwd: null stats/workspace");
    RU3D_REQUIRE(ws_bytes >= reduce_ws_bytes(y), "in_lrelu_bwd: workspace too small (%zu < %zu)", ws_bytes,
                 reduce_ws_bytes(y));
    RU3D_REQUIRE((int64_t)y->d * y->h * y->w < (1ll << 31), "in_lrelu_bwd: sample too large");
    if (dtype == RU3D_BF16 && in_small_mode(out, gpre_sum != nullptr, gout, y, dy, gpre)) {
        int rc = in_small_bwd_launch(gout, nullptr, 0, out, y, mean, scale, dy, gpre, ws, slope, zero_far, gpre_sum, as_stream(stream));
        if (rc || !dy_sum) return rc;
        return ru3d_channel_sum(dy, dy_sum, ws, ws_bytes, dtype, stream);
    }
    if (dtype == RU3D_F32)
        return in_bwd_impl<float>(gout, out, y, mean, scale, dy, gpre, ws, slope, zero_far, gpre_sum, dy_sum, as_stream(stream));
    if (dtype == RU3D_BF16)
        return in_bwd_impl<bf16>(gout, out, y, mean, scale, dy, gpre, ws, slope, zero_far, gpre_sum, dy_sum, as_stream(stream));
    return ru3d_fail(-1, "in_lrelu_bwd: bad dtype %d", dtype);
}

template <typename T>
static int in_bwd_apply_impl(const ru3d_tensor* gout, const ru3d_tensor* out, const float* mean, const float* scale,
                             const float* m12, const ru3d_tensor* dy, float slope, int zero_far, hipStream_t st) {
    const int64_t V = (int64_t)out->d * out->h * out->w;
    const int vec = pick_vec<T>(out->c, {gout, out, dy});
    ChanLoop ca = make_chanloop(V, out->c, vec, 16, out->n);
    dim3 grida(ca.chunks, out->n, (ca.G + ca.Gb - 1) / ca.Gb);
#define CALL(TT, VV)                                                                                                  \
    hipLaunchKernelGGL((in_lrelu_bwd_kernel<TT, VV, false>), grida, dim3(256), 0, st, (const TT*)gout->ptr, gout->ld, \
                       (const TT*)out->ptr, out->ld, (const TT*)out->ptr, out->ld, mean, scale, m12, (TT*)dy->ptr,    \
                       dy->ld, (TT*)0, 0, slope, zero_far, out->d, out->h, out->w, ca, out->c)
    DISPATCH_VEC(T, vec, CALL)
#undef CALL
    return ru3d_check_launch("in_lrelu_bwd_apply");
}

extern "C" int ru3d_in_lrelu_bwd_apply(const ru3d_tensor* gout, const ru3d_tensor* out, const float* mean,
                                       const float* scale, const float* m12, const ru3d_tensor* dy, float slope,
                                       int zero_far, int dtype, void* stream) {
    RU3D_FWD_F16(dtype, ru3d_in_lrelu_bwd_apply_f16(gout, out, mean, scale, m12, dy, slope, zero_far, dtype, stream));
    Ru3dDeviceGuard dev_guard(stream);
    RU3D_REQUIRE(tensor_ok(gout) && tensor_ok(out) && tensor_ok(dy), "in_lrelu_bwd_apply: bad tensor");
    RU3D_REQUIRE(same_shape(out, gout) && same_shape(out, dy), "in_lrelu_bwd_apply: shape mismatch");
    RU3D_REQUIRE(mean && scale && m12, "in_lrelu_bwd_apply: null stats");
    RU3D_REQUIRE((int64_t)out->d * out->h * out->w < (1ll << 31), "in_lrelu_bwd_apply: sample too large");
    if (dtype == RU3D_F32) return in_bwd_apply_impl<float>(gout, out, mean, scale, m12, dy, slope, zero_far, as_stream(stream));
    if (dtype == RU3D_BF16) return in_bwd_apply_impl<bf16>(gout, out, mean, scale, m12, dy, slope, zero_far, as_stream(stream));
    return ru3d_fail(-1, "in_lrelu_bwd_apply: bad dtype %d", dtype);
}

__global__ __launch_bounds__(256) void bn_pool_kernel(const double* __restrict__ part, int chunks, int C, int N,
                                                      const float* __restrict__ drop, double* __restrict__ pooled) {
    const int c = blockIdx.x * FIN_CX + threadIdx.x % FIN_CX;
    const bool ok = c < C;
    double s1 = 0.0, s2 = 0.0;
    for (int n = 0; n < N; n++) {
        double t1, t2;
        finalize_sums(part + (int64_t)n * chunks * C * 2, chunks, (int64_t)C * 2, ok ? c : 0, ok, t1, t2);
        if (ok && threadIdx.x < FIN_CX) {
            const double d = drop ? (double)drop[n * C + c] : 1.0;
            s1 += d * t1;
            s2 += d * d * t2;
        }
        __syncthreads();
    }
    if (ok && threadIdx.x < FIN_CX) {
        pooled[2 * c] = s1;
        pooled[2 * c + 1] = s2;
    }
}

__global__ void bn_m12_kernel(const double* __restrict__ pooled, int N, int C, double inv_count,
                              float* __restrict__ m12) {
    const int i = blockIdx.x * blockDim.x + threadIdx.x;
    if (i >= N * C) return;
    const int c = i % C;
    m12[2 * i] = (float)(pooled[2 * c] * inv_count);
    m12[2 * i + 1] = (float)(pooled[2 * c + 1] * inv_count);
}

#ifndef RU3D_STORAGE_F16
__global__ void bn_finalize_kernel(const double* __restrict__ pooled, int N, int C, int c_real, double inv_count,
                                   double unbias, const float* __restrict__ drop, const float* __restrict__ gamma,
                                   const float* __restrict__ beta, float eps, float momentum,
                                   float* __restrict__ running_mean, float* __restrict__ running_var,
                                   float* __restrict__ fscale, float* __restrict__ fshift, float* __restrict__ a,
                                   float* __restrict__ b) {
    const int i = blockIdx.x * blockDim.x + threadIdx.x;
    if (i >= N * C) return;
    const int n = i / C, c = i % C;
    const double m = pooled[2 * c] * inv_count;
    double var = pooled[2 * c + 1] * inv_count - m * m;
    if (var < 0.0) var = 0.0;
    const double r = 1.0 / sqrt(var + (double)eps);
    const double d = drop ? (double)drop[i] : 1.0;
    const bool real = c < c_real;
    const double g = (real && gamma) ? (double)gamma[c] : 1.0;
    const double be = (real && beta) ? (double)beta[c] : 0.0;
    a[i] = (float)(d * r);
    b[i] = (float)(-m * r);
    fscale[i] = (float)(g * d * r);
    fshift[i] = (float)(be - g * m * r);
    if (n == 0 && real && running_mean && running_var) {
// ... 409 lines not shown
```

### 3d-unet-renal-anatomy-extraction_amd/csrc/small_convs.hip

```cpp
#include "common.h"
#include "conv.h"

namespace RU3D_NS {

template <typename T>
__global__ __launch_bounds__(256) void stem_fwd_kernel(const T* __restrict__ x, const T* __restrict__ w,
                                                       const float* __restrict__ bias, T* __restrict__ y, ConvGeom g) {
    extern __shared__ float wl[];
    const int Cout = g.Cout;
    for (int i = threadIdx.x; i < 27 * Cout; i += 256) wl[i] = to_f32<T>(w[(i / Cout) * g.CoutPad + (i % Cout)]);
    for (int i = threadIdx.x; i < Cout; i += 256) wl[27 * Cout + i] = bias ? bias[i] : 0.f;
    __syncthreads();
    const int groups = Cout / 8;
    const int64_t total = (int64_t)g.N * g.Do * g.Ho * g.Wo * groups;
    const int64_t gid = (int64_t)blockIdx.x * 256 + threadIdx.x;
    if (gid >= total) return;
    const int cg = (int)(gid % groups);
    const int64_t vo = gid / groups;
    const int ow = (int)(vo % g.Wo);
    int64_t t = vo / g.Wo;
    const int oh = (int)(t % g.Ho);
    t /= g.Ho;
    const int od = (int)(t % g.Do);
    const int n = (int)(t / g.Do);
// ... 463 lines not shown
        const int tiles_h = (g.Ho + 7) / 8, tiles_w = (g.Wo + 31) / 32;
        const int64_t ntiles = (int64_t)g.N * g.Do * tiles_h * tiles_w;
        if (ntiles <= 0x7fffffff) {
            float* bias_part = db ? (float*)ws + (size_t)blocks * 27 * g.Cout : nullptr;
            hipLaunchKernelGGL(stem_wgrad_mfma_kernel, dim3(blocks, g.Cout / 32), dim3(256), 0, st, (const bf16*)x,
                               (const bf16*)dy, (float*)ws, g, tiles_h, tiles_w, (int)ntiles, bias_part);
            int rc = ru3d_check_launch("stem_wgrad_mfma");
            if (rc) return rc;
            rc = wgrad_reduce_launch((const float*)ws, dw, blocks, 27, 1, g.Cout, g.s_o, g.s_i, st);
            if (rc || !db) return rc;
            return wgrad_reduce_launch(bias_part, db, blocks, 1, 1, g.Cout, 1, 1, st);
        }
    }
    const int chunks = stem_chunks(g);
    dim3 grid(chunks, g.Cout / 32);
    if (dtype == RU3D_F32)
        hipLaunchKernelGGL(stem_wgrad_kernel<float>, grid, dim3(256), 0, st, (const float*)x, (const float*)dy,
                           (float*)ws, g);
    else
        hipLaunchKernelGGL(stem_wgrad_kernel<bf16>, grid, dim3(256), 0, st, (const bf16*)x, (const bf16*)dy,
                           (float*)ws, g);
    int rc = ru3d_check_launch("stem_wgrad");
    if (rc) return rc;
    return wgrad_reduce_launch((const float*)ws, dw, chunks, 27, 1, g.Cout, g.s_o, g.s_i, st);
}

#define HEAD_SPAN 4096
template <typename T, int VEC>
__global__ __launch_bounds__(256) void head_wgrad_kernel(const T* __restrict__ x, const T* __restrict__ dy,
                                                         float* __restrict__ part, WgradGeom g) {
    __shared__ float sh[256][VEC * 4 + 1];
    const int G = g.Cin / VEC;
    const int vpb = 256 / G;
    const int tid = threadIdx.x;
    const int cg = tid % G, vl = tid / G;
    const bool active = vl < vpb;
    const int64_t P = (int64_t)g.N * g.Do * g.Ho * g.Wo;
    const int64_t p0 = (int64_t)blockIdx.x * HEAD_SPAN;
    int64_t p1 = p0 + HEAD_SPAN;
    if (p1 > P) p1 = P;
    float acc[VEC][4];
#pragma unroll
    for (int i = 0; i < VEC; i++)
#pragma unroll
        for (int c = 0; c < 4; c++) acc[i][c] = 0.f;
    if (active) {
        constexpr int WU = 4;
        for (int64_t p = p0 + vl; p < p1; p += (int64_t)WU * vpb) {
            float xv[WU][VEC], dv[WU][4];
#pragma unroll
            for (int u = 0; u < WU; u++) {
                const int64_t pu = p + (int64_t)u * vpb;
                const bool ok = pu < p1;
                const int64_t pp = ok ? pu : p0;
                load_vec<T, VEC>(x + pp * g.ldx + cg * VEC, xv[u]);
#pragma unroll
                for (int c = 0; c < 4; c++) dv[u][c] = (ok && c < g.Cout) ? to_f32<T>(dy[pp * g.lddy + c]) : 0.f;
            }
#pragma unroll
            for (int u = 0; u < WU; u++)
#pragma unroll
                for (int i = 0; i < VEC; i++)
#pragma unroll
                    for (int c = 0; c < 4; c++) acc[i][c] = fmaf(xv[u][i], dv[u][c], acc[i][c]);
        }
    }
#pragma unroll
    for (int i = 0; i < VEC; i++)
#pragma unroll
        for (int c = 0; c < 4; c++) sh[tid][i * 4 + c] = active ? acc[i][c] : 0.f;
    __syncthreads();
    if (vl == 0) {
#pragma unroll
        for (int i = 0; i < VEC; i++)
            for (int c = 0; c < g.Cout; c++) {
                float s = 0.f;
                for (int l = 0; l < vpb; l++) s += sh[l * G + cg][i * 4 + c];
                part[((int64_t)blockIdx.x * g.Cin + cg * VEC + i) * g.Cout + c] = s;
            }
    }
}

constexpr int HB_U = 4;
__global__ __launch_bounds__(256) void head_bwd_kernel(const bf16* __restrict__ a, int lda, const float* __restrict__ dlog,
                                                       int ldd, const float* __restrict__ w, int cin_real, int Cin, int Cout,
                                                       bf16* __restrict__ dx, int lddx, float* __restrict__ part, int64_t P) {
    __shared__ float sh[256][33];
    const int G = Cin / 8, vpb = 256 / G;
    const int tid = threadIdx.x, cg = tid % G, vl = tid / G;
    float wr[4][8];
#pragma unroll
    for (int c = 0; c < 4; c++)
#pragma unroll
        for (int j = 0; j < 8; j++) {
            const int ci = cg * 8 + j;
            wr[c][j] = (c < Cout && ci < cin_real) ? (float)(bf16)w[c * cin_real + ci] : 0.f;
        }
    float aw[4][8], ab[4];
#pragma unroll
    for (int c = 0; c < 4; c++) {
        ab[c] = 0.f;
#pragma unroll
        for (int j = 0; j < 8; j++) aw[c][j] = 0.f;
    }
    const int64_t stride = (int64_t)gridDim.x * vpb;
    for (int64_t p0 = (int64_t)blockIdx.x * vpb + vl; p0 < P; p0 += HB_U * stride) {
        bf16x8 xv[HB_U];
        float dv[HB_U][4];
#pragma unroll
        for (int u = 0; u < HB_U; u++) {
            const int64_t p = p0 + u * stride;
            const bool ok = p < P;
            const int64_t pp = ok ? p : p0;
            xv[u] = *reinterpret_cast<const bf16x8*>(a + pp * lda + cg * 8);
#pragma unroll
            for (int c = 0; c < 4; c++) dv[u][c] = (ok && c < Cout) ? (float)(bf16)dlog[pp * ldd + c] : 0.f;
        }
#pragma unroll
        for (int u = 0; u < HB_U; u++) {
            const int64_t p = p0 + u * stride;
            float o[8];
#pragma unroll
            for (int j = 0; j < 8; j++) o[j] = 0.f;
#pragma unroll
            for (int c = 0; c < 4; c++) {
#pragma unroll
                for (int j = 0; j < 8; j++) {
                    o[j] = fmaf(dv[u][c], wr[c][j], o[j]);
                    aw[c][j] = fmaf((float)xv[u][j], dv[u][c], aw[c][j]);
                }
                ab[c] += dv[u][c];
            }
            if (p < P) store_vec<bf16, 8>(dx + p * lddx + cg * 8, o);
        }
    }
#pragma unroll
    for (int c = 0; c < 4; c++)
#pragma unroll
        for (int j = 0; j < 8; j++) sh[tid][c * 8 + j] = aw[c][j];
    sh[tid][32] = 0.f;
    __syncthreads();
    float* pp = part + (int64_t)blockIdx.x * (4 * Cin + 4);
    for (int e = tid; e < 4 * Cin; e += 256) {
        const int c = e / Cin, ci = e % Cin, g8 = ci / 8, j = ci % 8;
        float s = 0.f;
        for (int l = 0; l < vpb; l++) s += sh[l * G + g8][c * 8 + j];
        pp[e] = s;
    }
    __syncthreads();
    if (cg == 0) {
#pragma unroll
        for (int c = 0; c < 4; c++) sh[vl][c] = ab[c];
    }
    __syncthreads();
    if (tid < 4) {
        float s = 0.f;
        for (int l = 0; l < vpb; l++) s += sh[l][tid];
        pp[4 * Cin + tid] = s;
    }
}

__global__ __launch_bounds__(256) void head_bwd_finalize_kernel(const float* __restrict__ part, int blocks, int Cin,
                                                                int cin_real, int Cout, float* __restrict__ dw,
                                                                float* __restrict__ db) {
    const int e = blockIdx.x * 4 + (threadIdx.x >> 6), lane = threadIdx.x & 63;
    const int row = 4 * Cin + 4;
    if (e >= row) return;
    double acc = 0.0;
    for (int b = lane; b < blocks; b += 64) acc += (double)part[(int64_t)b * row + e];
    acc = wave_sum_d(acc);
    if (lane) return;
    if (e < 4 * Cin) {
        const int c = e / Cin, ci = e % Cin;
        if (c < Cout && ci < cin_real) dw[c * cin_real + ci] = (float)acc;
    } else if (e - 4 * Cin < Cout && db) {
        db[e - 4 * Cin] = (float)acc;
    }
}

static int head_bwd_blocks(int64_t P, int Cin) {
    const int vpb = 256 / (Cin / 8);
    int64_t b = (P + (int64_t)vpb * HB_U - 1) / ((int64_t)vpb * HB_U);
    return (int)(b < 2048 ? (b < 1 ? 1 : b) : 2048);
}

bool head_bwd_eligible(int Cin, int Cout, int dtype) {
    static const int mode = getenv("RU3D_HEAD_FUSED") ? atoi(getenv("RU3D_HEAD_FUSED")) : 1;
    const int G = Cin / 8;
    return mode && dtype == RU3D_BF16 && Cout >= 1 && Cout <= 4 && (Cin % 8) == 0 && G >= 1 && G <= 64 && (G & (G - 1)) == 0;
}

size_t head_bwd_ws_bytes(int64_t P, int Cin) { return (size_t)head_bwd_blocks(P, Cin) * (4 * Cin + 4) * sizeof(float); }

int head_bwd_launch(const void* a, int lda, const float* dlog, int ldd, const float* w, int cin_real, int Cin, int Cout,
                    void* dx, int lddx, float* dw, float* db, void* ws, int64_t P, hipStream_t st) {
    const int blocks = head_bwd_blocks(P, Cin);
    hipLaunchKernelGGL(head_bwd_kernel, dim3(blocks), dim3(256), 0, st, (const bf16*)a, lda, dlog, ldd, w, cin_real, Cin, Cout,
                       (bf16*)dx, lddx, (float*)ws, P);
    int rc = ru3d_check_launch("head_bwd");
    if (rc) return rc;
    const int vals = 4 * Cin + 4;
    hipLaunchKernelGGL(head_bwd_finalize_kernel, dim3((vals + 3) / 4), dim3(256), 0, st, (const float*)ws, blocks, Cin,
                       cin_real, Cout, dw, db);
    return ru3d_check_launch("head_bwd_finalize");
}

bool head_wgrad_eligible(const WgradGeom& g, int dtype) {
    const int vec = dtype == RU3D_BF16 ? 8 : 4;
    return g.k == 1 && g.stride == 1 && g.Cout <= 4 && (g.Cin % vec) == 0 && (g.Cin / vec) <= 256 &&
           (g.ldx % vec) == 0;
}

static int head_chunks(const WgradGeom& g) {
    const int64_t P = (int64_t)g.N * g.Do * g.Ho * g.Wo;
    return (int)((P + HEAD_SPAN - 1) / HEAD_SPAN);
}

size_t head_wgrad_ws_bytes(const WgradGeom& g) { return (size_t)head_chunks(g) * g.Cin * g.Cout * sizeof(float); }

int head_wgrad_launch(const void* x, const void* dy, float* dw, void* ws, size_t ws_bytes, const WgradGeom& g,
                      int dtype, hipStream_t st) {
    if (!ws || ws_bytes < head_wgrad_ws_bytes(g)) return ru3d_fail(-1, "head_wgrad: workspace too small");
    if (((uintptr_t)x) % 16) return ru3d_fail(-1, "head_wgrad: x must be 16-byte aligned");
    const int chunks = head_chunks(g);
    if (dtype == RU3D_F32)
        hipLaunchKernelGGL((head_wgrad_kernel<float, 4>), dim3(chunks), dim3(256), 0, st, (const float*)x,
                           (const float*)dy, (float*)ws, g);
    else
        hipLaunchKernelGGL((head_wgrad_kernel<bf16, 8>), dim3(chunks), dim3(256), 0, st, (const bf16*)x,
                           (const bf16*)dy, (float*)ws, g);
    int rc = ru3d_check_launch("head_wgrad");
    if (rc) return rc;
    return wgrad_reduce_launch((const float*)ws, dw, chunks, 1, g.Cin, g.Cout, g.s_o, g.s_i, st);
}

}
```

### 3d-unet-renal-anatomy-extraction_amd/network.py

```python
import os

import torch
import torch.nn as nn

import _native as N
import _ops as ops

_DEFAULT_DTYPE = {"fp32": torch.float32, "float32": torch.float32, "bf16": torch.bfloat16,
                  "bfloat16": torch.bfloat16, "fp16": torch.float16, "float16": torch.float16,
                  "half": torch.float16}[os.environ.get("RU3D_DTYPE", "fp32").lower()]


_STORAGE_DTYPES = (torch.float32, torch.bfloat16, torch.float16)


def set_compute_dtype(model, dtype):
    if dtype not in _STORAGE_DTYPES:
        raise ValueError("compute dtype must be one of %s" % (_STORAGE_DTYPES,))
    for m in model.modules():
        if isinstance(m, Unet):
            m.compute_dtype = dtype
            m._configure_native()
    return model

# ... 255 lines not shown
        if not self.attention and isinstance(self.conv_trans, ConvTrans3D):
            return self.conv_trans(x, skip, link)
        if (self.attention and isinstance(self.conv_trans, ConvTrans3D) and self.att_gate._native and x.is_cuda
                and (self.conv_trans._native or (self.conv_trans._bn_eval and _bn_on_device(self)))):
            up = self.conv_trans(x)
            return ops.AttGateFn.apply(skip, up, self.att_gate.conv.weight, self.att_gate.conv.bias,
                                       self.conv_trans._pad)
        x = self.conv_trans(x)
        if self.attention:
            skip = self.att_gate(skip, x)
        return torch.cat((x, skip), dim=1)


class ResBlock(nn.Module):

    def __init__(self, in_channels, out_channels, stride=1, conv_op=nn.Conv3d,
                 conv_kwargs={'kernel_size': 3, 'padding': 1},
                 dropout_op=nn.Dropout3d, dropout_kwargs={'p': 0.5, 'inplace': True},
                 norm_op=nn.InstanceNorm3d, norm_kwargs={},
                 nonlin_op=nn.LeakyReLU, nonlin_kwargs={'inplace': True}):
        super().__init__()
        self.in_channels = in_channels
        self.out_channels = out_channels
        self.stride = stride
        self.conv1 = conv_op(in_channels, out_channels, stride=stride, **conv_kwargs)
        self.conv2 = conv_op(out_channels, out_channels, **conv_kwargs)
        self.dropout = dropout_op(**dropout_kwargs) if dropout_op else None
        self.norm = norm_op(out_channels, **norm_kwargs)
        self.nonlin = nonlin_op(**nonlin_kwargs)
        self.skip_conv = conv_op(in_channels, out_channels, kernel_size=1, stride=stride)
        self._native = (_is_plain_conv3(self.conv1) and _is_plain_conv3(self.conv2)
                        and _is_plain_conv1(self.skip_conv) and _is_plain_in(self.norm)
                        and _is_plain_lrelu(self.nonlin)
                        and (self.dropout is None or type(self.dropout) is nn.Dropout3d))
        self._bn_eval = (_is_plain_conv3(self.conv1) and _is_plain_conv3(self.conv2) and _is_plain_conv1(self.skip_conv)
                         and _is_plain_bn(self.norm) and _is_plain_lrelu(self.nonlin))
        self._forced_keep = None
        self._pad = False
        self._in_segs = 1
        self._checkpoint = False

    @property
    def uses_skip_conv(self):
        return self.in_channels != self.out_channels or self.stride != 1

    def _drop_scale(self, x, planar=False):
        if self.dropout is None or not self.training:
            return None
        p = float(self.dropout.p)
        n = x.shape[0] // 2 if planar else x.shape[0]
        c = ops.cpad(self.out_channels) if self._pad else self.out_channels
        if self._forced_keep is not None:
            keep = self._forced_keep.to(device=x.device, dtype=torch.float32).reshape(n, -1)
            if keep.shape[1] != c:
                keep = torch.nn.functional.pad(keep, (0, c - keep.shape[1]), value=1.0)
            return (keep.reshape(-1) / (1.0 - p)).contiguous()
        if p == 0.0:
            return None
        pooled = ops.take_dropout(n, c, p)
        return pooled if pooled is not None else ops.dropout_scale(n, c, p, x.device)

    def _drop_spec(self, n):
        if (not self._native or self.dropout is None or not self.training or self._forced_keep is not None
                or float(self.dropout.p) == 0.0):
            return None
        return (n, ops.cpad(self.out_channels) if self._pad else self.out_channels, float(self.dropout.p))

    def _pack_specs(self):
        w1, w2 = self.conv1.weight, self.conv2.weight
        cout, cin = w1.shape[0], w1.shape[1]
        cout_seg = cout if self._pad else 0
        cin_seg = (cin // self._in_segs) if self._pad else 0
        specs = [(w1, N.ROLE_CONV_FWD, self.stride, cout_seg, cin_seg), (w1, N.ROLE_CONV_DGRAD, self.stride, cout_seg, cin_seg),
                 (w2, N.ROLE_CONV_FWD, 1, cout_seg, cout_seg), (w2, N.ROLE_CONV_DGRAD, 1, cout_seg, cout_seg)]
        biases = [self.conv1.bias, self.conv2.bias]
        if self.uses_skip_conv:
            ws = self.skip_conv.weight
            specs += [(ws, N.ROLE_CONV_FWD, self.stride, cout_seg, cin_seg), (ws, N.ROLE_CONV_DGRAD, self.stride, cout_seg, cin_seg)]
            biases.append(self.skip_conv.bias)
        if cout_seg:
            specs += [(b, N.ROLE_BIAS, 1, cout_seg, 0) for b in biases if b is not None]
        return specs

    def forward(self, x, in_link=None, out_link=None, planar=False):
        if self._native and x.is_cuda:
            skip_w = self.skip_conv.weight if self.uses_skip_conv else None
            skip_b = self.skip_conv.bias if self.uses_skip_conv else None
            return ops.ResBlockFn.apply(x, self.conv1.weight, self.conv1.bias, self.conv2.weight, self.conv2.bias,
                                        skip_w, skip_b, self.stride, self._drop_scale(x, planar),
                                        self._in_segs if self._pad else 0,
                                        self._checkpoint and torch.is_grad_enabled(), in_link, out_link, planar)
        if self._native:
            N.require_device(x, "ResBlock input")
        if self._bn_eval and x.is_cuda and _inference_mode(self):
            return self._forward_bn_eval(x)
        if (self._bn_eval and x.is_cuda and self.training and _bn_native_train()
                and (self.dropout is None or type(self.dropout) is nn.Dropout3d)):
            skip_w = self.skip_conv.weight if self.uses_skip_conv else None
            skip_b = self.skip_conv.bias if self.uses_skip_conv else None
            return ops.ResBlockBNFn.apply(x, self.conv1.weight, self.conv1.bias, self.conv2.weight, self.conv2.bias,
                                          skip_w, skip_b, self.norm.weight, self.norm.bias, self.stride,
                                          self._drop_scale(x), self._in_segs if self._pad else 0, self.norm)
        skip = self.skip_conv(x) if self.uses_skip_conv else x
        x = self.conv1(x)
        if self.dropout:
            x = self.dropout(x)
        x = self.nonlin(self.norm(x))
        x = self.conv2(x)
        return self.nonlin(self.norm(x) + skip)


def _resblock_bn_eval(self, x):
    x = ops.as_grad(x, x.dtype)
    sd = x.dtype
    cout, cin = self.conv1.weight.shape[0], self.conv1.weight.shape[1]
    cin_seg = ops.seg_of(cin, x.shape[1], self._in_segs) if self._pad else 0
    cout_seg = cout if self._pad else 0
    cp = ops.padded_dim(cout, cout_seg)
    specs = [(self.conv1.weight, N.ROLE_CONV_FWD, self.stride, cout_seg, cin_seg),
             (self.conv2.weight, N.ROLE_CONV_FWD, 1, cout_seg, cout_seg)]
    if self.uses_skip_conv:
        specs.append((self.skip_conv.weight, N.ROLE_CONV_FWD, self.stride, cout_seg, cin_seg))
    nw = len(specs)
    biases = [self.conv1.bias, self.conv2.bias, self.skip_conv.bias if self.uses_skip_conv else None]
    if cout_seg:
        specs += [(b, N.ROLE_BIAS, 1, cout_seg, 0) for b in biases if b is not None]
    packs = ops.pack_weights(specs, sd)
    if cout_seg:
        it = iter(packs[nw:])
        biases = [(ops._f32_view(next(it), cp) if b is not None else None) for b in biases]
    mean, scale = _bn_eval_stats(self.norm, x.shape[0], cp)
    y1 = ops.conv_fwd(x, packs[0], biases[0], cp, 3, self.stride)
    a1 = ops.in_lrelu_fwd(y1, mean, scale)
    y2 = ops.conv_fwd(a1, packs[1], biases[1], cp, 3, 1)
    skip = ops.conv_fwd(x, packs[2], biases[2], cp, 1, self.stride) if self.uses_skip_conv else x
    return ops.in_lrelu_fwd(y2, mean, scale, res=skip)


ResBlock._forward_bn_eval = _resblock_bn_eval


class ResBlockStack(nn.Module):
    def __init__(self, in_channels, out_channels, stride=1, num_stacks=2, conv_op=nn.Conv3d,
                 conv_kwargs={'kernel_size': 3, 'padding': 1},
                 dropout_op=nn.Dropout3d, dropout_kwargs={'p': 0.5, 'inplace': True},
                 norm_op=nn.InstanceNorm3d, norm_kwargs={},
                 nonlin_op=nn.LeakyReLU, nonlin_kwargs={'inplace': True}):
        super().__init__()
        common = dict(conv_op=conv_op, conv_kwargs=conv_kwargs, dropout_op=dropout_op,
                      dropout_kwargs=dropout_kwargs, norm_op=norm_op, norm_kwargs=norm_kwargs,
                      nonlin_op=nonlin_op, nonlin_kwargs=nonlin_kwargs)
        self.res_blocks = nn.ModuleList(
            ResBlock(in_channels if i == 0 else out_channels, out_channels, stride=stride if i == 0 else 1,
                     **common) for i in range(num_stacks))

    def forward(self, x, out_link=None):
        last = len(self.res_blocks) - 1
        for i, blk in enumerate(self.res_blocks):
            x = blk(x, out_link=out_link) if (i == last and out_link is not None) else blk(x)
        return x


class Unet(nn.Module):

    def __init__(self, in_channels, out_channels, paired_features,
                 pool_block=MaxPoolBlock, pool_kwargs={}, pool_kwargs_fn=none_fn,
                 up_block=UpConcat, up_kwargs={}, up_kwargs_fn=none_fn,
                 encode_block=ConvBlockStack, encode_kwargs={}, encode_kwargs_fn=none_fn,
                 decode_block=ConvBlockStack, decode_kwargs={}, decode_kwargs_fn=none_fn,
                 conv_op=nn.Conv3d, deep_supervision=0):
        super().__init__()
        num_pairs = len(paired_features)
        assert (num_pairs % 2) == 1, 'Number of paired features must be odd number.'
        self.num_pool = num_pairs // 2
# ... 93 lines not shown
        return torch.float32

    def _stem(self, x):
        if self._native_io and x.is_cuda:
            sd = self._storage_dtype()
            return ops.ConvFn.apply(x, self.conv.weight, self.conv.bias, 1, sd, sd, False, self._pad)
        if self._native_io:
            N.require_device(x, "Unet input")
        return self.conv(x)

    def _head(self, x):
        if self._native_io and x.is_cuda:
            return ops.ConvFn.apply(x, self.fc.weight, self.fc.bias, 1, x.dtype, torch.float32, self._pad, False)
        return self.fc(x)

    def _supervised_levels(self):
        return getattr(self, "deep_supervision", 0) if self.training else 0

    def _aux_head(self, level, x):
        head = self.ds_heads[level - 1]
        if self._native_io and x.is_cuda:
            return ops.ConvFn.apply(x, head.weight, head.bias, 1, x.dtype, torch.float32, self._pad, False)
        return head(x)

    def _prepack(self):
        sd = self._storage_dtype()
        cs = self.conv.weight.shape[0] if self._pad else 0
        specs = [(self.conv.weight, N.ROLE_CONV_FWD, 1, cs, 0)]
        if cs and self.conv.bias is not None:
            specs.append((self.conv.bias, N.ROLE_BIAS, 1, cs, 0))
        for blk in self._native_chain() or []:
            specs += blk._pack_specs()
        ci = self.fc.weight.shape[1] if self._pad else 0
        specs += [(self.fc.weight, N.ROLE_CONV_FWD, 1, 0, ci), (self.fc.weight, N.ROLE_CONV_DGRAD, 1, 0, ci)]
        for level in range(1, self._supervised_levels()):
            w = self.ds_heads[level - 1].weight
            ci = w.shape[1] if self._pad else 0
            specs += [(w, N.ROLE_CONV_FWD, 1, 0, ci), (w, N.ROLE_CONV_DGRAD, 1, 0, ci)]
        ops.prepack(specs, sd)

    def _set_bn_pad(self, pad):
        if pad != self._pad:
            self._pad = pad
            for blk in self._bn_blocks:
                blk._pad = pad

    def forward(self, x):
        if self._bn_blocks is not None:
            self._set_bn_pad(self._pad_bn and x.is_cuda and _bn_on_device(self))
        linked = self._linked and x.is_cuda
        if linked and torch.is_grad_enabled() and self._storage_dtype() != torch.float32:
            self._prepack()
        x = self._stem(x)
        skips, links = [], []
        if linked and self.training:
            order = []
            for i in range(self.num_pool):
                order += [self.encode_blocks[i], self.pool_blocks[i]]
            order += [self.encode_blocks[-1]]
            for i in reversed(range(self.num_pool)):
                order += [self.decode_blocks[i]]
            specs = []
            for m in order:
                for blk in (m.res_blocks if isinstance(m, ResBlockStack) else [m]):
                    sp = blk._drop_spec(x.shape[0]) if isinstance(blk, ResBlock) else None
                    if sp is not None:
                        specs.append(sp)
            ops.prefill_dropout(specs, x.device)
        for i in range(self.num_pool):
            link = None
            if linked:
                cu = self.up_blocks[i].conv_trans.out_channels
                cd = self.decode_blocks[i].out_channels if isinstance(self.decode_blocks[i], ResBlock) else 0
                link = ops.SkipLink(ops.cpad(cu) if self._pad else cu, ops.cpad(cd) if self._pad else cd)
                x = self.encode_blocks[i](x, out_link=link)
            else:
                x = self.encode_blocks[i](x)
            skips.append(x)
            links.append(link)
            x = self.pool_blocks[i](x, in_link=link) if linked else self.pool_blocks[i](x)
        x = self.encode_blocks[-1](x)
        levels = self._supervised_levels()
        aux = {}
        for i in reversed(range(self.num_pool)):
            x = self.up_blocks[i](x, skips[i], links[i]) if linked else self.up_blocks[i](x, skips[i])
            if linked and getattr(links[i], "planar_out", False):
                x = self.decode_blocks[i](x, planar=True)
            else:
                x = self.decode_blocks[i](x)
            if 1 <= i < levels:
                aux[i] = self._aux_head(i, x)
        ops._DROP_POOL.clear()
        if levels:
            return [self._head(x)] + [aux[l] for l in range(1, levels)]
        return self._head(x)


def _stacks_by_level(level):
    return {'num_stacks': max(level, 1)}


class _UnetWrapper(nn.Module):
    def forward(self, x):
        return self.net(x)


class ResUnet3D(_UnetWrapper):

    def __init__(self, num_pool=4, num_features=30, in_channels=1, out_channels=1, deep_supervision=0):
        super().__init__()
        self.num_pool = num_pool
        self.num_features = num_features
        self.in_channels = in_channels
        self.out_channels = out_channels
        self.net = Unet(in_channels=in_channels, out_channels=out_channels,
                        paired_features=generate_paired_features(num_pool, num_features),
                        pool_block=ResBlock, pool_kwargs={'stride': 2},
                        encode_block=ResBlockStack, encode_kwargs_fn=_stacks_by_level,
                        decode_block=ResBlock, deep_supervision=deep_supervision)


class ResAttrUnet3D(_UnetWrapper):

    def __init__(self, num_pool=4, num_features=30, in_channels=1, out_channels=1, deep_supervision=0):
        super().__init__()
        self.num_pool = num_pool
        self.num_features = num_features
        self.in_channels = in_channels
        self.out_channels = out_channels
        self.net = Unet(in_channels=in_channels, out_channels=out_channels,
                        paired_features=generate_paired_features(num_pool, num_features),
                        pool_block=ResBlock, pool_kwargs={'stride': 2}, up_kwargs={'attention': True},
                        encode_block=ResBlockStack, encode_kwargs_fn=_stacks_by_level,
                        decode_block=ResBlock, deep_supervision=deep_supervision)


class ResAttrUnet3D2(_UnetWrapper):

    def __init__(self, in_channels=1, out_channels=1, deep_supervision=0):
        super().__init__()
        self.in_channels = in_channels
        self.out_channels = out_channels
        widths = [30, 60, 120, 240, 320]
        plan = [[c, c] for c in widths] + [[320, 320]] + [[c, c] for c in reversed(widths)]
        self.net = Unet(in_channels=in_channels, out_channels=out_channels, paired_features=plan,
                        pool_block=ResBlock, pool_kwargs={'stride': 2}, up_kwargs={'attention': True},
                        encode_block=ResBlockStack, encode_kwargs_fn=_stacks_by_level,
                        decode_block=ResBlock, deep_supervision=deep_supervision)


class ResAttrBNUnet3D(_UnetWrapper):

    def __init__(self, num_pool=4, num_features=30, in_channels=1, out_channels=1, deep_supervision=0):
        super().__init__()
        self.num_pool = num_pool
        self.num_features = num_features
        self.in_channels = in_channels
        self.out_channels = out_channels
        bn = {'norm_op': nn.BatchNorm3d}
        self.net = Unet(in_channels=in_channels, out_channels=out_channels,
                        paired_features=generate_paired_features(num_pool, num_features),
                        pool_block=ResBlock, pool_kwargs={'stride': 2, **bn},
                        up_kwargs={'attention': True, **bn},
                        encode_block=ResBlockStack, encode_kwargs=bn, encode_kwargs_fn=_stacks_by_level,
                        decode_block=ResBlock, decode_kwargs=bn, deep_supervision=deep_supervision)
```

### include/ru3d.h

```cpp
#ifndef RU3D_H
#define RU3D_H

#include <stddef.h>
#include <stdint.h>

#ifdef __cplusplus
extern "C" {
#endif

#define RU3D_VERSION 201

enum { RU3D_F32 = 0, RU3D_BF16 = 1, RU3D_F16 = 2 };

enum { RU3D_LABEL_I64 = 0, RU3D_LABEL_U8 = 1 };

enum {
    RU3D_ROLE_CONV_FWD = 0,
    RU3D_ROLE_CONV_DGRAD = 1,
    RU3D_ROLE_CONVT_FWD = 2,
    RU3D_ROLE_CONVT_DGRAD = 3,
    RU3D_ROLE_BIAS = 4
};

enum {
    RU3D_LOSS_HYBIRD = 0,
    RU3D_LOSS_DICELOSS = 1,
    RU3D_LOSS_FOCAL = 2,
    RU3D_LOSS_DICE = 3
};

typedef struct ru3d_tensor {
    void* ptr;
    int32_t n, d, h, w;
    int32_t c;
    int32_t ld;
    int32_t cseg;
    int64_t seg_stride;
} ru3d_tensor;

int ru3d_version(void);
const char* ru3d_last_error(void);
void ru3d_launch_log_begin(void);
const char* ru3d_launch_log_end(void);

size_t ru3d_packed_weight_bytes(int cout, int cin, int k, int stride, int role, int dtype);
int ru3d_pack_weight(const float* src, void* dst, int cout, int cin, int k, int stride, int role, int dtype,
                     void* stream);

#define RU3D_PACK_MAX 40
typedef struct ru3d_pack_item {
    const float* src;
    void* dst;
    int32_t cout, cin, k, stride, role;
    int32_t cout_seg, cin_seg;
} ru3d_pack_item;
int ru3d_pack_weights(const ru3d_pack_item* items, int count, int dtype, void* stream);

int ru3d_unpad_weight_grad(const float* src, float* dst, int cout, int cin, int taps, int cout_seg, int cin_seg,
                           void* stream);

size_t ru3d_conv3d_workspace_bytes(const ru3d_tensor* x, const ru3d_tensor* y, int k, int stride, int dtype);
int ru3d_conv3d_fwd(const ru3d_tensor* x, const void* w_packed, const float* bias, const ru3d_tensor* res,
                    const ru3d_tensor* y, int k, int stride, int dtype, int y_dtype, void* ws,
                    size_t ws_bytes, void* stream);
size_t ru3d_conv3d_fwd_in_workspace_bytes(const ru3d_tensor* x, const ru3d_tensor* y, int k, int stride, int dtype);
int ru3d_conv3d_fwd_in(const ru3d_tensor* x, const void* w_packed, const float* bias, const ru3d_tensor* y, int k,
                       int stride, int dtype, const float* drop_scale, float* mean, float* scale, void* ws,
                       size_t ws_bytes, float eps, void* stream);
size_t ru3d_conv3d_fwd_in_lrelu_workspace_bytes(const ru3d_tensor* x, const ru3d_tensor* y, int k, int stride, int dtype);
int ru3d_conv3d_fwd_in_lrelu(const ru3d_tensor* x, const void* w_packed, const float* bias, const ru3d_tensor* y, int k,
                             int stride, int dtype, const float* drop_scale, float* mean, float* scale,
                             const ru3d_tensor* res, const ru3d_tensor* out, float slope, void* ws, size_t ws_bytes,
                             float eps, void* stream);
int ru3d_planar_concat_supported(int n, int d, int h, int w, int cseg, int cout, int dtype);
int ru3d_conv3d_dgrad(const ru3d_tensor* dy, const void* w_packed, const ru3d_tensor* res,
                      const ru3d_tensor* dx, int k, int stride, int dtype, void* ws, size_t ws_bytes,
                      void* stream);
int ru3d_conv3d_s1_dgrad_pair_supported(const ru3d_tensor* dy, const ru3d_tensor* dy2, const ru3d_tensor* dx, int dtype);
int ru3d_conv3d_s1_dgrad_pair(const ru3d_tensor* dy, const void* w3_packed, const ru3d_tensor* dy2, const void* w1_packed,
                              const ru3d_tensor* dx, int dtype, void* stream);
int ru3d_conv3d_s2_pair_fwd_in_supported(const ru3d_tensor* x, const ru3d_tensor* y3, const ru3d_tensor* y1, int dtype);
size_t ru3d_conv3d_s2_pair_fwd_in_workspace_bytes(const ru3d_tensor* x, const ru3d_tensor* y3, int dtype);
int ru3d_conv3d_s2_pair_fwd_in(const ru3d_tensor* x, const void* w3_packed, const float* b3, const ru3d_tensor* y3,
                               const void* w1_packed, const float* b1, const ru3d_tensor* y1, const float* drop_scale,
                               float* mean, float* scale, void* ws, size_t ws_bytes, float eps, int dtype, void* stream);
int ru3d_conv3d_s2_dgrad_pair_supported(const ru3d_tensor* dy, const ru3d_tensor* dy2, const ru3d_tensor* res,
                                        const ru3d_tensor* dx, int dtype);
int ru3d_conv3d_s2_dgrad_pair(const ru3d_tensor* dy, const void* w3_packed, const ru3d_tensor* dy2,
                              const void* w1_packed, const ru3d_tensor* res, const ru3d_tensor* dx, int dtype,
                              void* stream);
size_t ru3d_conv3d_wgrad_workspace_bytes(const ru3d_tensor* x, const ru3d_tensor* dy, int k, int stride, int dtype);
int ru3d_conv3d_wgrad(const ru3d_tensor* x, const ru3d_tensor* dy, float* dw, void* ws, size_t ws_bytes,
                      int k, int stride, int dtype, void* stream);

int ru3d_conv3d_wgrad_pair_supported(const ru3d_tensor* x, const ru3d_tensor* dy, const ru3d_tensor* dy2, int stride, int dtype);
size_t ru3d_conv3d_wgrad_pair_workspace_bytes(const ru3d_tensor* x, const ru3d_tensor* dy, const ru3d_tensor* dy2, int stride,
                                              int dtype);
int ru3d_conv3d_wgrad_pair(const ru3d_tensor* x, const ru3d_tensor* dy, const ru3d_tensor* dy2, float* dw, float* dw2,
                           void* ws, size_t ws_bytes, int stride, int dtype, void* stream);
size_t ru3d_conv3d_wgrad_bias_workspace_bytes(const ru3d_tensor* x, const ru3d_tensor* dy, int k, int stride, int dtype);
int ru3d_conv3d_wgrad_bias(const ru3d_tensor* x, const ru3d_tensor* dy, float* dw, float* db, void* ws, size_t ws_bytes,
                           int k, int stride, int dtype, void* stream);
int ru3d_head_bwd_supported(const ru3d_tensor* x, const ru3d_tensor* dlogits, const ru3d_tensor* dx, int dtype);
size_t ru3d_head_bwd_workspace_bytes(const ru3d_tensor* x, int dtype);
int ru3d_head_bwd(const ru3d_tensor* x, const ru3d_tensor* dlogits, const float* weight, int cin_real, const ru3d_tensor* dx,
                  float* dw, float* db, void* ws, size_t ws_bytes, int dtype, void* stream);

int ru3d_convtranspose3d_k3s2p1_fwd(const ru3d_tensor* x, const void* w_packed, const float* bias,
                                    const ru3d_tensor* y, int dtype, void* stream);
size_t ru3d_convtranspose3d_k3s2p1_fwd_in_workspace_bytes(const ru3d_tensor* x, const ru3d_tensor* y, int dtype);
int ru3d_convtranspose3d_k3s2p1_fwd_in(const ru3d_tensor* x, const void* w_packed, const float* bias,
                                       const ru3d_tensor* y, float* mean, float* scale, void* ws, size_t ws_bytes,
                                       float eps, int dtype, void* stream);
int ru3d_convtranspose3d_k3s2p1_dgrad(const ru3d_tensor* dy, const void* w_packed, const ru3d_tensor* dx,
                                      int dtype, void* stream);
size_t ru3d_convtranspose3d_k3s2p1_wgrad_workspace_bytes(const ru3d_tensor* x, const ru3d_tensor* dy, int dtype);
int ru3d_convtranspose3d_k3s2p1_wgrad(const ru3d_tensor* x, const ru3d_tensor* dy, float* dw, void* ws,
                                      size_t ws_bytes, int dtype, void* stream);

size_t ru3d_reduce_workspace_bytes(const ru3d_tensor* t);
int ru3d_instnorm_stats(const ru3d_tensor* y, const float* drop_scale, float* mean, float* scale,
                        void* ws, size_t ws_bytes, float eps, int dtype, void* stream);
int ru3d_skip1x1_in_lrelu_fwd_supported(const ru3d_tensor* x, const ru3d_tensor* y, const ru3d_tensor* out, int dtype);
int ru3d_skip1x1_in_lrelu_fwd(const ru3d_tensor* x, const void* w_packed, const float* bias, const ru3d_tensor* y,
                              const float* mean, const float* scale, const ru3d_tensor* out, float slope, int dtype,
                              void* stream);
int ru3d_in_lrelu_fwd(const ru3d_tensor* y, const float* mean, const float* scale, const ru3d_tensor* res,
                      const ru3d_tensor* out, float slope, int dtype, void* stream);
int ru3d_in_lrelu_bwd(const ru3d_tensor* gout, const ru3d_tensor* out, const ru3d_tensor* y, const float* mean,
                      const float* scale, const ru3d_tensor* dy, const ru3d_tensor* gpre, void* ws,
                      size_t ws_bytes, float slope, int zero_far, float* gpre_sum, float* dy_sum, int dtype,
                      void* stream);
int ru3d_channel_sum(const ru3d_tensor* t, float* out, void* ws, size_t ws_bytes, int dtype, void* stream);
int ru3d_dropout3d_scale(float* scale, int count, float p, uint64_t seed, uint64_t offset, void* stream);
int ru3d_dropout3d_scale_dev(float* scale, int count, float p, uint64_t seed, uint64_t offset,
                             const uint64_t* offset_base, void* stream);

int ru3d_pointwise(int op, const ru3d_tensor* a, const ru3d_tensor* b, const ru3d_tensor* c, const ru3d_tensor* o1,
                   const ru3d_tensor* o2, float slope, int dtype, void* stream);

int ru3d_copy_channels(const ru3d_tensor* src, const ru3d_tensor* dst, int dtype, void* stream);
int ru3d_add(const ru3d_tensor* a, const ru3d_tensor* b, const ru3d_tensor* dst, int dtype, void* stream);
int ru3d_cast_f32(const ru3d_tensor* src, const ru3d_tensor* dst, int dst_dtype, void* stream);
int ru3d_ncdhw_to_ndhwc(const float* src, const ru3d_tensor* dst, int dtype, void* stream);
int ru3d_ndhwc_to_ncdhw(const ru3d_tensor* src, float* dst, int dtype, void* stream);

size_t ru3d_loss_state_bytes(int num_classes);
size_t ru3d_loss_state_bad_labels_offset(void);
size_t ru3d_loss_workspace_bytes(int n, int64_t v, int num_classes);
int ru3d_loss_fwd(const float* logits, int64_t stride_n, int64_t stride_c, int64_t stride_v, const void* labels,
                  int label_dtype, int n, int64_t v, int num_classes, int kind, float gamma, const float* weight_v,
                  float alpha, float beta, float smooth, void* state, float* loss_out, void* ws, size_t ws_bytes,
                  void* stream);
int ru3d_loss_bwd(const float* logits, int64_t stride_n, int64_t stride_c, int64_t stride_v, const void* labels,
                  int label_dtype, int n, int64_t v, int num_classes, float gamma, const void* state,
                  const float* grad_out, void* dlogits, int dlogits_dtype, void* stream);
int ru3d_tversky(const float* p, const float* g, int64_t count, float alpha, float beta, float smooth,
                 float* out, void* ws, size_t ws_bytes, void* stream);

int ru3d_predict_accumulate(const ru3d_tensor* logits, int dtype, int sample, float* acc, float* cnt, int X, int Y,
                            int Z, int ox, int oy, int oz, void* stream);
int ru3d_predict_merge(const float* acc, const float* cnt, int X, int Y, int Z, int num_classes, int cx, int cy,
                       int cz, int sx, int sy, int sz, int one_hot, void* out, void* stream);
#define RU3D_PREDICT_MAX_BATCH 16
int ru3d_predict_gather(const float* vol, int X, int Y, int Z, int cin, const int32_t* windows, int count,
                        const ru3d_tensor* dst, void* stream);
int ru3d_predict_accumulate_weighted(const ru3d_tensor* logits, int dtype, int sample, int flip, const float* gx,
                                     const float* gy, const float* gz, float* acc, float* cnt, int X, int Y, int Z,
                                     int ox, int oy, int oz, void* stream);

size_t ru3d_components_workspace_bytes(int X, int Y, int Z);
int ru3d_label_components(const uint8_t* mask, int X, int Y, int Z, int32_t* labels, int32_t* count_dev, void* ws,
                          size_t ws_bytes, void* stream);
int ru3d_component_stats(const int32_t* labels, int X, int Y, int Z, int count, int32_t* sizes, int32_t* boxes,
                         void* stream);
size_t ru3d_filter_components_workspace_bytes(int count);
int ru3d_filter_components(const int32_t* labels, int X, int Y, int Z, int count, const int32_t* sizes, int threshold,
                           uint8_t* mask_inout, int32_t* labels_out, int32_t* kept_dev, void* ws, size_t ws_bytes,
                           void* stream);
int ru3d_region_accumulate(const float* prob, int rx, int ry, int rz, int num_classes, int bx, int by, int bz,
                           double* total, int32_t* hits, int X, int Y, int Z, void* stream);
int ru3d_cascade_merge(const double* total, const int32_t* hits, int X, int Y, int Z, int num_classes, uint8_t* out,
                       void* stream);

enum { RU3D_MASK_NE = 0, RU3D_MASK_EQ = 1, RU3D_MASK_GT = 2, RU3D_MASK_GE = 3 };
enum { RU3D_MORPH_ERODE = 0, RU3D_MORPH_DILATE = 1 };
#define RU3D_MORPH_MAX_EXTENT 15
#define RU3D_MORPH_MAX_ROWS 225
typedef struct ru3d_morph_row {
    int8_t dx, dy;
    uint16_t zmask;
} ru3d_morph_row;
size_t ru3d_mask_bytes(int X, int Y, int Z);
int ru3d_mask_pack(const uint8_t* src, int X, int Y, int Z, int op, int value, uint64_t* bits, void* stream);
int ru3d_mask_unpack(const uint64_t* bits, int X, int Y, int Z, int value, int paint, uint8_t* dst, void* stream);
int ru3d_binary_morph(const uint64_t* src, uint64_t* dst, int X, int Y, int Z, int op, const ru3d_morph_row* rows,
                      int num_rows, int border_value, void* stream);
int ru3d_confusion_counts(const uint8_t* pred, const uint8_t* label, int64_t n, int num_classes, int64_t* table,
                          void* stream);

int ru3d_threshold_bbox(const float* image, int X, int Y, int Z, int C, float threshold, int32_t* box, int64_t* count,
                        void* stream);
size_t ru3d_masked_sample_workspace_bytes(int X, int Y, int Z);
int ru3d_masked_sample(const float* image, int X, int Y, int Z, int C, int channel, const void* label, int label_dtype,
                       int stride, float* out, int64_t capacity, int64_t* count, void* ws, size_t ws_bytes, void* stream);
#define RU3D_ORDER_STATS_MAX_RANKS 8
size_t ru3d_order_stats_workspace_bytes(void);
int ru3d_order_stats(const float* values, int64_t n, const int64_t* ranks, int num_ranks, float* out, void* ws,
                     size_t ws_bytes, void* stream);
// ... 254 lines not shown
```

Measured before the change: 273.6 million voxels/s.

## Fuse final 1x1 head conv into last decoder ResBlock tail forward and backward

```diff
diff --git a/3d-unet-renal-anatomy-extraction_amd/_native.py b/3d-unet-renal-anatomy-extraction_amd/_native.py
--- a/3d-unet-renal-anatomy-extraction_amd/_native.py
+++ b/3d-unet-renal-anatomy-extraction_amd/_native.py
@@ -137,6 +137,11 @@
     "ru3d_in_lrelu_fwd": (_i, [_P, _vp, _vp, _P, _P, _f, _i, _vp]),
     "ru3d_skip1x1_in_lrelu_fwd_supported": (_i, [_P, _P, _P, _i]),
     "ru3d_skip1x1_in_lrelu_fwd": (_i, [_P, _vp, _vp, _P, _vp, _vp, _P, _f, _i, _vp]),
+    "ru3d_skip1x1_in_lrelu_head_fwd_supported": (_i, [_P, _P, _P, _P, _i]),
+    "ru3d_skip1x1_in_lrelu_head_fwd": (_i, [_P, _vp, _vp, _P, _vp, _vp, _P, _vp, _vp, _P, _f, _i, _vp]),
+    "ru3d_head_in_bwd_supported": (_i, [_P, _P, _P, _P, _P, _i]),
+    "ru3d_head_in_bwd_workspace_bytes": (_sz, [_P, _i]),
+    "ru3d_head_in_bwd": (_i, [_P, _P, _vp, _i, _P, _vp, _vp, _P, _P, _vp, _vp, _vp, _vp, _sz, _f, _i, _vp]),
     "ru3d_in_lrelu_bwd": (_i, [_P, _P, _P, _vp, _vp, _P, _P, _vp, _sz, _f, _i, _vp, _vp, _i, _vp]),
     "ru3d_in_lrelu_bwd_apply": (_i, [_P, _P, _vp, _vp, _vp, _P, _f, _i, _i, _vp]),
     "ru3d_conv3d_dgrad_in_bwd_workspace_bytes": (_sz, [_P, _P, _i, _i, _i]),
diff --git a/3d-unet-renal-anatomy-extraction_amd/_ops.py b/3d-unet-renal-anatomy-extraction_amd/_ops.py
--- a/3d-unet-renal-anatomy-extraction_amd/_ops.py
+++ b/3d-unet-renal-anatomy-extraction_amd/_ops.py
@@ -537,6 +537,48 @@
     return out
 
 
+def head_tail_mode():
+    return os.environ.get("RU3D_HEAD_TAIL", "1")
+
+
+def skip1x1_in_lrelu_head_fwd(x, pw, bias, y, mean, scale, head_pw, head_bias, head_cout):
+    code = N.dtype_code(y.dtype)
+    if code == N.F32 or head_cout > 4:
+        return None
+    n, c, d, h, w = y.shape
+    out = N.new_act(n, c, d, h, w, y.dtype, y.device)
+    logits = N.new_act(n, head_cout, d, h, w, torch.float32, y.device)
+    dx, dy, do, dl = desc(x), desc(y), desc(out), desc(logits)
+    if not N.lib.ru3d_skip1x1_in_lrelu_head_fwd_supported(ref(dx), ref(dy), ref(do), ref(dl), code):
+        return None
+    check(N.lib.ru3d_skip1x1_in_lrelu_head_fwd(ref(dx), ptr(pw), ptr(_bias(bias)), ref(dy), ptr(mean), ptr(scale), ref(do),
+                                               ptr(head_pw), ptr(_bias(head_bias)), ref(dl), LRELU_SLOPE, code, stream()),
+          "skip1x1_in_lrelu_head_fwd")
+    return out, logits
+
+
+def head_in_bwd(z, gy, weight, want_bias, y, mean, scale, key=None):
+    if gy.dtype != torch.float32 or z.dtype == torch.float32 or not N.is_ndhwc(gy) or weight.dtype != torch.float32:
+        return None
+    n, c, d, h, w = z.shape
+    dy = N.new_act(n, c, d, h, w, z.dtype, z.device)
+    gpre = N.new_act(n, c, d, h, w, z.dtype, z.device)
+    dz, dg, dyy, dp, ddy = desc(z), desc(gy), desc(y), desc(gpre), desc(dy)
+    code = N.dtype_code(z.dtype)
+    if not N.lib.ru3d_head_in_bwd_supported(ref(dz), ref(dg), ref(dyy), ref(dp), ref(ddy), code):
+        return None
+    cout, cin = weight.shape[0], weight.shape[1]
+    dw = _grad_out(key, (cout, cin, 1, 1, 1), z.device)
+    db = torch.empty(cout, dtype=torch.float32, device=z.device) if want_bias else None
+    gsum = torch.empty(c, dtype=torch.float32, device=z.device)
+    ws = N.workspace(N.lib.ru3d_head_in_bwd_workspace_bytes(ref(dz), code), z.device)
+    wd = weight.detach()
+    check(N.lib.ru3d_head_in_bwd(ref(dz), ref(dg), ptr(wd if wd.is_contiguous() else wd.contiguous()), cin, ref(dyy),
+                                 ptr(mean), ptr(scale), ref(dp), ref(ddy), ptr(dw), ptr(db), ptr(gsum), ptr(ws), ws.numel(),
+                                 LRELU_SLOPE, code, stream()), "head_in_bwd")
+    return dy, gpre, gsum, dw, db
+
+
 def in_lrelu_bwd(gout, out, y, mean, scale, want_gpre=False, zero_far=False, want_gpre_sum=False, dy_sum=None):
     n, c, d, h, w = y.shape
     dy = N.new_act(n, c, d, h, w, y.dtype, y.device)
@@ -918,7 +960,7 @@
 
     @staticmethod
     def forward(ctx, x, w1, b1, w2, b2, ws, bs, stride, drop_scale, pad=0, checkpoint=False, in_link=None,
-                out_link=None, planar=False):
+                out_link=None, planar=False, head_w=None, head_b=None):
         sd = x.dtype
         x = N.to_ndhwc(x)
         xt = x
@@ -965,9 +1007,19 @@
         z = None
         tail = (fused is None and ws is not None and stride == 1 and out_link is None and sd != torch.float32
                 and (x.shape[1], cout_p) in ((64, 32), (128, 64)) and n_ * d_ * h_ * w_ >= 65536)
+        logits = head_pack = None
+        if head_w is not None:
+            if head_w.shape[1] != cout or head_w.shape[2] != 1 or out_link is not None:
+                raise N.Ru3dError("ResBlock: the head must be a 1x1x1 conv on the block's %d output channels" % cout)
+            head_pack = pack_weights([(head_w, N.ROLE_CONV_FWD, 1, 0, cout_seg)], sd)[0]
         if tail:
             y2, mean2, scale2 = conv_fwd_in(a1, pw2, b2, cout_p, 3, 1)
-            z = skip1x1_in_lrelu_fwd(x, packs[2], bs, y2, mean2, scale2)
+            both = (skip1x1_in_lrelu_head_fwd(x, packs[2], bs, y2, mean2, scale2, head_pack, head_b, head_w.shape[0])
+                    if (head_w is not None and head_tail_mode() != "bwd") else None)
+            if both is not None:
+                z, logits = both
+            else:
+                z = skip1x1_in_lrelu_fwd(x, packs[2], bs, y2, mean2, scale2)
             if z is None:
                 z = in_lrelu_fwd(y2, mean2, scale2, res=conv_fwd(x, packs[2], bs, cout_p, 1, stride), out=zout)
         else:
@@ -978,13 +1030,19 @@
             else:
                 skip = x
             y2, mean2, scale2, z = conv_fwd_in_act(a1, pw2, b2, cout_p, 3, 1, res=skip, out=zout)
+        if head_w is not None and logits is None:
+            logits = conv_fwd(z, head_pack, head_b, head_w.shape[0], 1, 1, out_dtype=torch.float32)
         bwd = packs[nfwd:nw] + [None] * 3
+        hsave = head_w if train else None
         if checkpoint and train:
             ctx.save_for_backward(xt, None, None, None, z, mean1, scale1, mean2, scale2, bwd[0], bwd[1], bwd[2],
-                                  pw1, pw2, b1, b2)
+                                  pw1, pw2, b1, b2, hsave)
         else:
             ctx.save_for_backward(xt, y1, a1, y2, z, mean1, scale1, mean2, scale2, bwd[0], bwd[1], bwd[2],
-                                  None, None, None, None)
+                                  None, None, None, None, hsave)
+        ctx.head = head_w is not None
+        ctx.head_bias = head_b is not None
+        ctx.hkey = head_w.data_ptr() if (head_w is not None and not cout_seg) else None
         ctx.planar = bool(planar)
         ctx.dims = (cout, cin, cout_seg, cin_seg)
         ctx.stride = stride
@@ -995,26 +1053,52 @@
         ctx.in_link = in_link if (in_link is not None and ws is not None) else None
         if in_link is not None:
             in_link.fused_grad = ctx.in_link is not None and need_gx
-        return z
+        return logits if head_w is not None else z
+
+    @staticmethod
+    def _head_backward(ctx, gy, z, head_w, y2, mean2, scale2):
+        cout, cin, cout_seg, cin_seg = ctx.dims
+        sd = z.dtype
+        want_b = ctx.head_bias and ctx.needs_input_grad[15]
+        fused = head_in_bwd(z, gy, head_w, want_b, y2, mean2, scale2, key=ctx.hkey) if head_tail_mode() != "fwd" else None
+        if fused is not None:
+            return fused
+        hb = head_bwd(z, gy, head_w, want_b, key=ctx.hkey)
+        if hb is not None:
+            gz, ghw, ghb = hb
+        else:
+            gy = as_grad(gy, sd)
+            hcout = head_w.shape[0]
+            ghw = unpad_wgrad(conv_wgrad(z, gy, 1, 1, key=ctx.hkey), hcout, cout, 0, cout_seg)
+            ghb = channel_sum(gy)[:hcout] if want_b else None
+            pwd = pack_weights([(head_w, N.ROLE_CONV_DGRAD, 1, 0, cout_seg)], sd)[0]
+            gz = conv_dgrad(gy, pwd, tuple(z.shape), 1, 1)
+        dy2, gpre, gbs_sum = in_lrelu_bwd(gz, z, y2, mean2, scale2, want_gpre=True, want_gpre_sum=True)
+        return dy2, gpre, gbs_sum, ghw, ghb
 
     @staticmethod
     def backward(ctx, gz):
-        (x, y1, a1, y2, z, mean1, scale1, mean2, scale2, pw2d, pw1d, pwsd, pw1, pw2, b1, b2) = ctx.saved_tensors
+        (x, y1, a1, y2, z, mean1, scale1, mean2, scale2, pw2d, pw1d, pwsd, pw1, pw2, b1, b2, head_w) = ctx.saved_tensors
         cout, cin, cout_seg, cin_seg = ctx.dims
         cout_p = padded_dim(cout, cout_seg)
         sd = x.dtype
         dev = x.device
         stride = ctx.stride
-        gz = as_grad(gz, sd)
+        if not ctx.head:
+            gz = as_grad(gz, sd)
         if ctx.planar:
             x = N.Split(x)
         if y1 is None:
             y1 = conv_fwd(x, pw1, b1, cout_p, 3, stride)
             a1 = in_lrelu_fwd(y1, mean1, scale1)
             y2 = conv_fwd(a1, pw2, b2, cout_p, 3, 1)
-        dy2, gpre, gbs_sum = in_lrelu_bwd(gz, z, y2, mean2, scale2, want_gpre=True, want_gpre_sum=True)
+        ghw = ghb = None
+        if ctx.head:
+            dy2, gpre, gbs_sum, ghw, ghb = ResBlockFn._head_backward(ctx, gz, z, head_w, y2, mean2, scale2)
+        else:
+            dy2, gpre, gbs_sum = in_lrelu_bwd(gz, z, y2, mean2, scale2, want_gpre=True, want_gpre_sum=True)
         del y2
-        return ResBlockFn._backward_tail(ctx, x, a1, y1, dy2, gpre, gbs_sum, mean1, scale1, pw2d, pw1d, pwsd)
+        return ResBlockFn._backward_tail(ctx, x, a1, y1, dy2, gpre, gbs_sum, mean1, scale1, pw2d, pw1d, pwsd) + (ghw, ghb)
 
     @staticmethod
     def _backward_tail(ctx, x, a1, y1, dy2, gpre, gbs_sum, mean1, scale1, pw2d, pw1d, pwsd):
diff --git a/3d-unet-renal-anatomy-extraction_amd/csrc/api.hip b/3d-unet-renal-anatomy-extraction_amd/csrc/api.hip
--- a/3d-unet-renal-anatomy-extraction_amd/csrc/api.hip
+++ b/3d-unet-renal-anatomy-extraction_amd/csrc/api.hip
@@ -437,6 +437,27 @@
     return skip1x1_fused_launch(x, w_packed, bias, y, mean, scale, out, slope, as_stream(stream));
 }
 
+extern "C" int ru3d_skip1x1_in_lrelu_head_fwd_supported(const ru3d_tensor* x, const ru3d_tensor* y, const ru3d_tensor* out,
+                                                        const ru3d_tensor* logits, int dtype) {
+    RU3D_FWD_F16(dtype, ru3d_skip1x1_in_lrelu_head_fwd_supported_f16(x, y, out, logits, dtype));
+    return skip1x1_head_fused_eligible(x, y, out, logits, dtype) ? 1 : 0;
+}
+
+extern "C" int ru3d_skip1x1_in_lrelu_head_fwd(const ru3d_tensor* x, const void* w_packed, const float* bias,
+                                              const ru3d_tensor* y, const float* mean, const float* scale,
+                                              const ru3d_tensor* out, const void* head_w_packed, const float* head_bias,
+                                              const ru3d_tensor* logits, float slope, int dtype, void* stream) {
+    RU3D_FWD_F16(dtype, ru3d_skip1x1_in_lrelu_head_fwd_f16(x, w_packed, bias, y, mean, scale, out, head_w_packed, head_bias,
+                                                           logits, slope, dtype, stream));
+    Ru3dDeviceGuard dev_guard(stream);
+    RU3D_REQUIRE(w_packed && mean && scale && head_w_packed, "skip1x1_in_lrelu_head_fwd: null argument");
+    RU3D_REQUIRE(skip1x1_head_fused_eligible(x, y, out, logits, dtype),
+                 "skip1x1_in_lrelu_head_fwd: shapes have no fused kernel (ask ru3d_skip1x1_in_lrelu_head_fwd_supported first)");
+    RU3D_REQUIRE((((uintptr_t)head_w_packed) % 8) == 0, "skip1x1_in_lrelu_head_fwd: the head's pack must be 8-byte aligned");
+    return skip1x1_fused_launch(x, w_packed, bias, y, mean, scale, out, slope, as_stream(stream), head_w_packed, head_bias,
+                                logits);
+}
+
 extern "C" int ru3d_conv3d_s2_pair_fwd_in_supported(const ru3d_tensor* x, const ru3d_tensor* y3, const ru3d_tensor* y1, int dtype) {
     RU3D_FWD_F16(dtype, ru3d_conv3d_s2_pair_fwd_in_supported_f16(x, y3, y1, dtype));
     if (dtype != RU3D_BF16 || !tensor_ok(x) || !tensor_ok(y3) || !tensor_ok(y1)) return 0;
diff --git a/3d-unet-renal-anatomy-extraction_amd/csrc/conv.h b/3d-unet-renal-anatomy-extraction_amd/csrc/conv.h
--- a/3d-unet-renal-anatomy-extraction_amd/csrc/conv.h
+++ b/3d-unet-renal-anatomy-extraction_amd/csrc/conv.h
@@ -121,8 +121,11 @@
                         const void* w2, const float* bias2, void* y2, int ldy2, hipStream_t st);
 
 bool skip1x1_fused_eligible(const ru3d_tensor* x, const ru3d_tensor* y2, const ru3d_tensor* out, int dtype);
+bool skip1x1_head_fused_eligible(const ru3d_tensor* x, const ru3d_tensor* y2, const ru3d_tensor* out,
+                                 const ru3d_tensor* logits, int dtype);
 int skip1x1_fused_launch(const ru3d_tensor* x, const void* w, const float* bias, const ru3d_tensor* y2, const float* mean,
-                         const float* scale, const ru3d_tensor* out, float slope, hipStream_t st);
+                         const float* scale, const ru3d_tensor* out, float slope, hipStream_t st,
+                         const void* head_w = nullptr, const float* head_bias = nullptr, const ru3d_tensor* logits = nullptr);
 
 int in_small_mode(const ru3d_tensor* y, bool all_samples, const ru3d_tensor* a = nullptr, const ru3d_tensor* b = nullptr,
                   const ru3d_tensor* c = nullptr, const ru3d_tensor* d = nullptr);
diff --git a/3d-unet-renal-anatomy-extraction_amd/csrc/f16_names.h b/3d-unet-renal-anatomy-extraction_amd/csrc/f16_names.h
--- a/3d-unet-renal-anatomy-extraction_amd/csrc/f16_names.h
+++ b/3d-unet-renal-anatomy-extraction_amd/csrc/f16_names.h
@@ -40,6 +40,11 @@
     X(ru3d_in_lrelu_fwd) \
     X(ru3d_skip1x1_in_lrelu_fwd_supported) \
     X(ru3d_skip1x1_in_lrelu_fwd) \
+    X(ru3d_skip1x1_in_lrelu_head_fwd_supported) \
+    X(ru3d_skip1x1_in_lrelu_head_fwd) \
+    X(ru3d_head_in_bwd_supported) \
+    X(ru3d_head_in_bwd_workspace_bytes) \
+    X(ru3d_head_in_bwd) \
     X(ru3d_in_lrelu_bwd) \
     X(ru3d_channel_sum) \
     X(ru3d_copy_channels) \
@@ -94,6 +99,11 @@
 #define ru3d_in_lrelu_fwd ru3d_in_lrelu_fwd_f16
 #define ru3d_skip1x1_in_lrelu_fwd_supported ru3d_skip1x1_in_lrelu_fwd_supported_f16
 #define ru3d_skip1x1_in_lrelu_fwd ru3d_skip1x1_in_lrelu_fwd_f16
+#define ru3d_skip1x1_in_lrelu_head_fwd_supported ru3d_skip1x1_in_lrelu_head_fwd_supported_f16
+#define ru3d_skip1x1_in_lrelu_head_fwd ru3d_skip1x1_in_lrelu_head_fwd_f16
+#define ru3d_head_in_bwd_supported ru3d_head_in_bwd_supported_f16
+#define ru3d_head_in_bwd_workspace_bytes ru3d_head_in_bwd_workspace_bytes_f16
+#define ru3d_head_in_bwd ru3d_head_in_bwd_f16
 #define ru3d_in_lrelu_bwd ru3d_in_lrelu_bwd_f16
 #define ru3d_channel_sum ru3d_channel_sum_f16
 #define ru3d_copy_channels ru3d_copy_channels_f16
diff --git a/3d-unet-renal-anatomy-extraction_amd/csrc/fused_skip.hip b/3d-unet-renal-anatomy-extraction_amd/csrc/fused_skip.hip
--- a/3d-unet-renal-anatomy-extraction_amd/csrc/fused_skip.hip
+++ b/3d-unet-renal-anatomy-extraction_amd/csrc/fused_skip.hip
@@ -37,9 +37,13 @@
     float slope;
     int x_cseg;
     int64_t x_segstride;
+    const bf16x4* hw;
+    const float* hbias;
+    float* logits;
+    int hcout, ldl;
 };
 
-template <int CIN, int NPB>
+template <int CIN, int NPB, bool HEAD = false>
 __global__ __launch_bounds__(256) void skip1x1_in_lrelu_fwd_kernel(SkipArgs a) {
     constexpr int KS = CIN / 32;
     const int lane = threadIdx.x & 63;
@@ -59,6 +63,15 @@
     for (int pb = 0; pb < NPB; pb++)
 #pragma unroll
         for (int i = 0; i < 8; i++) bias8[pb][i] = a.bias ? a.bias[pb * 32 + 8 * g4 + i] : 0.f;
+
+    __shared__ bf16x4 hws[HEAD ? 32 * NPB : 1];
+    float hb = 0.f;
+    int hrow = 8 * g4;
+    if constexpr (HEAD) {
+        if (threadIdx.x < 32 * NPB) hws[threadIdx.x] = a.hw[threadIdx.x];
+        hb = (a.hbias && g4 < a.hcout) ? a.hbias[g4] : 0.f;
+        __syncthreads();
+    }
 
     const int64_t groups_per_sample = a.V / 16;
     const int64_t total = groups_per_sample * a.N;
@@ -102,6 +115,7 @@
                 acc[j >> 1][j & 1] = RU3D_MFMA_16X16X32(wreg[ks * NPB * 2 + j], xb[ks], acc[j >> 1][j & 1], 0, 0, 0);
             });
         });
+        float hsum[4];
 #pragma unroll
         for (int pb = 0; pb < NPB; pb++) {
             f32x4 a0 = acc[pb][0], a1 = acc[pb][1];
@@ -114,7 +128,28 @@
                 const float t = ((float)yv[pb][i] - mu[pb][i]) * sc[pb][i] + (float)sk[i];
                 o[i] = t > 0.f ? t : t * a.slope;
             }
-            *reinterpret_cast<bf16x8*>(a.out + vox * a.ldo + pb * 32 + 8 * g4) = __builtin_convertvector(o, bf16x8);
+            const bf16x8 zr = __builtin_convertvector(o, bf16x8);
+            *reinterpret_cast<bf16x8*>(a.out + vox * a.ldo + pb * 32 + 8 * g4) = zr;
+            if constexpr (HEAD) {
+                float hacc[4] = {0.f, 0.f, 0.f, 0.f};
+                asm volatile("" : "+v"(hrow));
+#pragma unroll
+                for (int i = 0; i < 8; i++) {
+                    const bf16x4 h = hws[pb * 32 + hrow + i];
+#pragma unroll
+                    for (int c = 0; c < 4; c++) hacc[c] = fmaf((float)zr[i], (float)h[c], hacc[c]);
+                }
+#pragma unroll
+                for (int c = 0; c < 4; c++) {
+                    hacc[c] += __shfl_xor(hacc[c], 16, 64);
+                    hacc[c] += __shfl_xor(hacc[c], 32, 64);
+                    hsum[c] = pb == 0 ? hacc[c] : hsum[c] + hacc[c];
+                }
+            }
+        }
+        if constexpr (HEAD) {
+            const float mine = g4 == 0 ? hsum[0] : (g4 == 1 ? hsum[1] : (g4 == 2 ? hsum[2] : hsum[3]));
+            if (g4 < a.hcout) a.logits[vox * a.ldl + g4] = mine + hb;
         }
     }
 }
@@ -135,8 +170,16 @@
     return (V % 16) == 0 && V * x->n >= 65536;
 }
 
+bool skip1x1_head_fused_eligible(const ru3d_tensor* x, const ru3d_tensor* y2, const ru3d_tensor* out,
+                                 const ru3d_tensor* logits, int dtype) {
+    if (!skip1x1_fused_eligible(x, y2, out, dtype) || !tensor_ok(logits)) return false;
+    if (logits->n != y2->n || logits->d != y2->d || logits->h != y2->h || logits->w != y2->w) return false;
+    return logits->c >= 1 && logits->c <= 4 && (((uintptr_t)logits->ptr) % 4) == 0;
+}
+
 int skip1x1_fused_launch(const ru3d_tensor* x, const void* w, const float* bias, const ru3d_tensor* y2, const float* mean,
-                         const float* scale, const ru3d_tensor* out, float slope, hipStream_t st) {
+                         const float* scale, const ru3d_tensor* out, float slope, hipStream_t st, const void* head_w,
+                         const float* head_bias, const ru3d_tensor* logits) {
     SkipArgs a;
     a.x = (const bf16*)x->ptr; a.w = (const bf16x8*)w; a.bias = bias; a.y2 = (const bf16*)y2->ptr;
     a.mean = mean; a.scale = scale; a.out = (bf16*)out->ptr;
@@ -146,10 +189,18 @@
     a.cout = y2->c;
     a.slope = slope;
     a.x_cseg = x->cseg; a.x_segstride = x->seg_stride;
+    a.hw = (const bf16x4*)head_w; a.hbias = head_bias;
+    a.logits = logits ? (float*)logits->ptr : nullptr;
+    a.hcout = logits ? logits->c : 0; a.ldl = logits ? logits->ld : 0;
     const int64_t groups = a.V / 16 * a.N;
     int64_t blocks = (groups + 3) / 4;
     const int64_t cap = 256 * 8;
     if (blocks > cap) blocks = cap;
+    if (logits) {
+        if (x->c == 64) hipLaunchKernelGGL((skip1x1_in_lrelu_fwd_kernel<64, 1, true>), dim3((unsigned)blocks), dim3(256), 0, st, a);
+        else hipLaunchKernelGGL((skip1x1_in_lrelu_fwd_kernel<128, 2, true>), dim3((unsigned)blocks), dim3(256), 0, st, a);
+        return ru3d_check_launch("skip1x1_in_lrelu_head_fwd");
+    }
     if (x->c == 64) hipLaunchKernelGGL((skip1x1_in_lrelu_fwd_kernel<64, 1>), dim3((unsigned)blocks), dim3(256), 0, st, a);
     else hipLaunchKernelGGL((skip1x1_in_lrelu_fwd_kernel<128, 2>), dim3((unsigned)blocks), dim3(256), 0, st, a);
     return ru3d_check_launch("skip1x1_in_lrelu_fwd");
diff --git a/3d-unet-renal-anatomy-extraction_amd/csrc/norm.hip b/3d-unet-renal-anatomy-extraction_amd/csrc/norm.hip
--- a/3d-unet-renal-anatomy-extraction_amd/csrc/norm.hip
+++ b/3d-unet-renal-anatomy-extraction_amd/csrc/norm.hip
@@ -592,6 +592,149 @@
     return ru3d_fail(-1, "in_lrelu_bwd: bad dtype %d", dtype);
 }
 
+template <int VEC>
+__global__ __launch_bounds__(256) void head_dz_reduce2_kernel(const float* __restrict__ dlog, int ldd,
+                                                              const float* __restrict__ w, int cin_real, int Cout,
+                                                              const bf16* __restrict__ b, int ldb,
+                                                              const bf16* __restrict__ c3, int ldc,
+                                                              const float* __restrict__ mean,
+                                                              const float* __restrict__ scale, float slope,
+                                                              double* __restrict__ part, ChanLoop cl, int C,
+                                                              bf16* __restrict__ gp_out, int ldgp) {
+    static_assert(VEC == 8, "head_bwd_kernel's piece: 8 channels a lane");
+    __shared__ double sh[2][256][4];
+    const int tid = threadIdx.x;
+    const int cgl = tid % cl.Gb, vl = tid / cl.Gb;
+    const int cg = blockIdx.z * cl.Gb + cgl;
+    const int n = blockIdx.y;
+    const bool active = (vl < cl.vpb) && (cg < cl.G);
+    float s1[VEC], s2[VEC];
+#pragma unroll
+    for (int i = 0; i < VEC; i++) s1[i] = s2[i] = 0.f;
+    if (active) {
+        float mu[VEC], sc[VEC], wr[4][VEC];
+#pragma unroll
+        for (int i = 0; i < VEC; i++) {
+            mu[i] = mean[n * C + cg * VEC + i];
+            sc[i] = scale[n * C + cg * VEC + i];
+            const int ci = cg * VEC + i;
+#pragma unroll
+            for (int c = 0; c < 4; c++)
+                wr[c][i] = (c < Cout && ci < cin_real) ? (float)(bf16)w[c * cin_real + ci] : 0.f;
+        }
+        const int v0 = blockIdx.x * cl.span;
+        int v1 = v0 + cl.span;
+        if (v1 > cl.V) v1 = cl.V;
+        for (int v = v0 + vl; v < v1; v += cl.vpb) {
+            const int64_t row = (int64_t)n * cl.V + v;
+            float dv[4], av[VEC], ov[VEC], yv[VEC], pv[VEC];
+#pragma unroll
+            for (int c = 0; c < 4; c++) dv[c] = c < Cout ? (float)(bf16)dlog[row * ldd + c] : 0.f;
+            load_vec<bf16, VEC>(b + row * ldb + cg * VEC, ov);
+            load_vec<bf16, VEC>(c3 + row * ldc + cg * VEC, yv);
+#pragma unroll
+            for (int i = 0; i < VEC; i++) av[i] = 0.f;
+#pragma unroll
+            for (int c = 0; c < 4; c++)
+#pragma unroll
+                for (int i = 0; i < VEC; i++) av[i] = fmaf(dv[c], wr[c][i], av[i]);
+#pragma unroll
+            for (int i = 0; i < VEC; i++) {
+                const float dz = to_f32<bf16>(from_f32<bf16>(av[i]));
+                float gp = ov[i] > 0.f ? dz : dz * slope;
+                gp = to_f32<bf16>(from_f32<bf16>(gp));
+                pv[i] = gp;
+                const float xh = (yv[i] - mu[i]) * sc[i];
+                s1[i] += gp;
+                s2[i] = fmaf(gp, xh, s2[i]);
+            }
+            store_vec<bf16, VEC>(gp_out + row * ldgp + cg * VEC, pv);
+        }
+    }
+#pragma unroll
+    for (int half = 0; half < 2; half++) {
+        __syncthreads();
+#pragma unroll
+        for (int i = 0; i < 4; i++) {
+            sh[0][tid][i] = active ? (double)s1[half * 4 + i] : 0.0;
+            sh[1][tid][i] = active ? (double)s2[half * 4 + i] : 0.0;
+        }
+        __syncthreads();
+        if (vl == 0 && cg < cl.G) {
+#pragma unroll
+            for (int i = 0; i < 4; i++) {
+                double t1 = 0.0, t2 = 0.0;
+                for (int l = 0; l < cl.vpb; l++) {
+                    t1 += sh[0][l * cl.Gb + cgl][i];
+                    t2 += sh[1][l * cl.Gb + cgl][i];
+                }
+                const int c = cg * VEC + half * 4 + i;
+                double* pp = part + (((int64_t)n * cl.chunks + blockIdx.x) * C + c) * 2;
+                pp[0] = t1;
+                pp[1] = t2;
+            }
+        }
+    }
+}
+
+static size_t head_in_red_bytes(const ru3d_tensor* z) { return ((reduce_ws_bytes(z) + 255) / 256) * 256; }
+
+extern "C" int ru3d_head_in_bwd_supported(const ru3d_tensor* z, const ru3d_tensor* dlogits, const ru3d_tensor* y,
+                                          const ru3d_tensor* gpre, const ru3d_tensor* dy, int dtype) {
+    RU3D_FWD_F16(dtype, ru3d_head_in_bwd_supported_f16(z, dlogits, y, gpre, dy, dtype));
+    if (!tensor_ok(z) || !tensor_ok(dlogits) || !tensor_ok(y) || !tensor_ok(gpre) || !tensor_ok(dy)) return 0;
+    if (z->n != dlogits->n || z->d != dlogits->d || z->h != dlogits->h || z->w != dlogits->w) return 0;
+    if (!same_shape(z, y) || !same_shape(z, gpre) || !same_shape(z, dy)) return 0;
+    if ((int64_t)z->d * z->h * z->w >= (1ll << 31) || (((uintptr_t)dlogits->ptr) % 4)) return 0;
+    if (pick_vec<bf16>(z->c, {z, y, gpre, dy}) != 8) return 0;
+    if (dtype == RU3D_BF16 && in_small_mode(z, true, gpre, y, dy, gpre)) return 0;
+    return head_bwd_eligible(z->c, dlogits->c, dtype) ? 1 : 0;
+}
+
+extern "C" size_t ru3d_head_in_bwd_workspace_bytes(const ru3d_tensor* z, int dtype) {
+    RU3D_FWD_F16(dtype, ru3d_head_in_bwd_workspace_bytes_f16(z, dtype));
+    if (!tensor_ok(z) || (z->c % 8)) return 0;
+    return head_in_red_bytes(z) + head_bwd_ws_bytes(nvox(z), z->c);
+}
+
+extern "C" int ru3d_head_in_bwd(const ru3d_tensor* z, const ru3d_tensor* dlogits, const float* weight, int cin_real,
+                                const ru3d_tensor* y, const float* mean, const float* scale, const ru3d_tensor* gpre,
+                                const ru3d_tensor* dy, float* dw, float* db, float* gpre_sum, void* ws, size_t ws_bytes,
+                                float slope, int dtype, void* stream) {
+    RU3D_FWD_F16(dtype, ru3d_head_in_bwd_f16(z, dlogits, weight, cin_real, y, mean, scale, gpre, dy, dw, db, gpre_sum, ws,
+                                             ws_bytes, slope, dtype, stream));
+    Ru3dDeviceGuard dev_guard(stream);
+    RU3D_REQUIRE(ru3d_head_in_bwd_supported(z, dlogits, y, gpre, dy, dtype),
+                 "head_in_bwd: shapes have no fused kernel (ask ru3d_head_in_bwd_supported first)");
+    RU3D_REQUIRE(weight && dw && mean && scale && ws && cin_real > 0 && cin_real <= z->c, "head_in_bwd: bad argument");
+    RU3D_REQUIRE(ws_bytes >= ru3d_head_in_bwd_workspace_bytes(z, dtype), "head_in_bwd: workspace too small");
+    hipStream_t st = as_stream(stream);
+    const int64_t V = (int64_t)z->d * z->h * z->w;
+    int rc = head_bwd_launch(z->ptr, z->ld, (const float*)dlogits->ptr, dlogits->ld, weight, cin_real, z->c, dlogits->c,
+                             nullptr, 0, dw, db, (char*)ws + head_in_red_bytes(z), nvox(z), st);
+    if (rc) return rc;
+    ChanLoop cl = make_chanloop(V, y->c, 8, 64, y->n);
+    dim3 grid(cl.chunks, y->n, (cl.G + cl.Gb - 1) / cl.Gb);
+    double* part = (double*)ws;
+    float* m12 = (float*)((char*)ws + (size_t)y->n * cl.chunks * y->c * 2 * sizeof(double));
+    hipLaunchKernelGGL((head_dz_reduce2_kernel<8>), grid, dim3(256), 0, st, (const float*)dlogits->ptr, dlogits->ld, weight,
+                       cin_real, dlogits->c, (const bf16*)z->ptr, z->ld, (const bf16*)y->ptr, y->ld, mean, scale, slope, part,
+                       cl, y->c, (bf16*)gpre->ptr, gpre->ld);
+    rc = ru3d_check_launch("head_in_bwd_reduce");
+    if (rc) return rc;
+    hipLaunchKernelGGL(bwd_finalize_kernel, dim3((y->c + FIN_CX - 1) / FIN_CX), dim3(256), 0, st, (const double*)part,
+                       cl.chunks, y->c, y->n, 1.0 / (double)V, m12, (double)V, gpre_sum);
+    rc = ru3d_check_launch("head_in_bwd_finalize");
+    if (rc) return rc;
+    ChanLoop ca = make_chanloop(V, y->c, 8, 16, y->n);
+    dim3 grida(ca.chunks, y->n, (ca.G + ca.Gb - 1) / ca.Gb);
+    hipLaunchKernelGGL((in_lrelu_bwd_kernel<bf16, 8, true, true>), grida, dim3(256), 0, st, (const bf16*)nullptr, 0,
+                       (const bf16*)nullptr, 0, (const bf16*)y->ptr, y->ld, mean, scale, (const float*)m12, (bf16*)dy->ptr,
+                       dy->ld, (bf16*)gpre->ptr, gpre->ld, slope, 0, y->d, y->h, y->w, ca, y->c, (const float*)nullptr,
+                       (const float*)nullptr, (double*)nullptr);
+    return ru3d_check_launch("head_in_bwd_apply");
+}
+
 template <typename T>
 static int in_bwd_apply_impl(const ru3d_tensor* gout, const ru3d_tensor* out, const float* mean, const float* scale,
                              const float* m12, const ru3d_tensor* dy, float slope, int zero_far, hipStream_t st) {
diff --git a/3d-unet-renal-anatomy-extraction_amd/csrc/small_convs.hip b/3d-unet-renal-anatomy-extraction_amd/csrc/small_convs.hip
--- a/3d-unet-renal-anatomy-extraction_amd/csrc/small_convs.hip
+++ b/3d-unet-renal-anatomy-extraction_amd/csrc/small_convs.hip
@@ -569,9 +569,10 @@
 }
 
 constexpr int HB_U = 4;
-__global__ __launch_bounds__(256) void head_bwd_kernel(const bf16* __restrict__ a, int lda, const float* __restrict__ dlog,
-                                                       int ldd, const float* __restrict__ w, int cin_real, int Cin, int Cout,
-                                                       bf16* __restrict__ dx, int lddx, float* __restrict__ part, int64_t P) {
+template <bool STORE_DX>
+__device__ __forceinline__ void head_bwd_body(const bf16* __restrict__ a, int lda, const float* __restrict__ dlog, int ldd,
+                                              const float* __restrict__ w, int cin_real, int Cin, int Cout,
+                                              bf16* __restrict__ dx, int lddx, float* __restrict__ part, int64_t P) {
     __shared__ float sh[256][33];
     const int G = Cin / 8, vpb = 256 / G;
     const int tid = threadIdx.x, cg = tid % G, vl = tid / G;
@@ -618,7 +619,7 @@
                 }
                 ab[c] += dv[u][c];
             }
-            if (p < P) store_vec<bf16, 8>(dx + p * lddx + cg * 8, o);
+            if (STORE_DX && p < P) store_vec<bf16, 8>(dx + p * lddx + cg * 8, o);
         }
     }
 #pragma unroll
@@ -645,6 +646,19 @@
         for (int l = 0; l < vpb; l++) s += sh[l][tid];
         pp[4 * Cin + tid] = s;
     }
+}
+
+__global__ __launch_bounds__(256) void head_bwd_kernel(const bf16* __restrict__ a, int lda, const float* __restrict__ dlog,
+                                                       int ldd, const float* __restrict__ w, int cin_real, int Cin, int Cout,
+                                                       bf16* __restrict__ dx, int lddx, float* __restrict__ part, int64_t P) {
+    head_bwd_body<true>(a, lda, dlog, ldd, w, cin_real, Cin, Cout, dx, lddx, part, P);
+}
+
+__global__ __launch_bounds__(256) void head_bwd_wgrad_kernel(const bf16* __restrict__ a, int lda,
+                                                             const float* __restrict__ dlog, int ldd,
+                                                             const float* __restrict__ w, int cin_real, int Cin, int Cout,
+                                                             float* __restrict__ part, int64_t P) {
+    head_bwd_body<false>(a, lda, dlog, ldd, w, cin_real, Cin, Cout, nullptr, 0, part, P);
 }
 
 __global__ __launch_bounds__(256) void head_bwd_finalize_kernel(const float* __restrict__ part, int blocks, int Cin,
@@ -682,9 +696,16 @@
 int head_bwd_launch(const void* a, int lda, const float* dlog, int ldd, const float* w, int cin_real, int Cin, int Cout,
                     void* dx, int lddx, float* dw, float* db, void* ws, int64_t P, hipStream_t st) {
     const int blocks = head_bwd_blocks(P, Cin);
-    hipLaunchKernelGGL(head_bwd_kernel, dim3(blocks), dim3(256), 0, st, (const bf16*)a, lda, dlog, ldd, w, cin_real, Cin, Cout,
-                       (bf16*)dx, lddx, (float*)ws, P);
-    int rc = ru3d_check_launch("head_bwd");
+    int rc;
+    if (dx) {
+        hipLaunchKernelGGL(head_bwd_kernel, dim3(blocks), dim3(256), 0, st, (const bf16*)a, lda, dlog, ldd, w, cin_real, Cin,
+                           Cout, (bf16*)dx, lddx, (float*)ws, P);
+        rc = ru3d_check_launch("head_bwd");
+    } else {
+        hipLaunchKernelGGL(head_bwd_wgrad_kernel, dim3(blocks), dim3(256), 0, st, (const bf16*)a, lda, dlog, ldd, w, cin_real,
+                           Cin, Cout, (float*)ws, P);
+        rc = ru3d_check_launch("head_bwd_wgrad");
+    }
     if (rc) return rc;
     const int vals = 4 * Cin + 4;
     hipLaunchKernelGGL(head_bwd_finalize_kernel, dim3((vals + 3) / 4), dim3(256), 0, st, (const float*)ws, blocks, Cin,
diff --git a/3d-unet-renal-anatomy-extraction_amd/network.py b/3d-unet-renal-anatomy-extraction_amd/network.py
--- a/3d-unet-renal-anatomy-extraction_amd/network.py
+++ b/3d-unet-renal-anatomy-extraction_amd/network.py
@@ -361,14 +361,35 @@
             specs += [(b, N.ROLE_BIAS, 1, cout_seg, 0) for b in biases if b is not None]
         return specs
 
-    def forward(self, x, in_link=None, out_link=None, planar=False):
+    def takes_head(self, x, head, planar=False):
+        if ops.head_tail_mode() == "0":
+            return False
+        if not (self._native and x.is_cuda and x.dtype != torch.float32 and self.uses_skip_conv and self.stride == 1):
+            return False
+        if (self._checkpoint and torch.is_grad_enabled()) or self._forward_hooks or self._forward_pre_hooks:
+            return False
+        if not (_is_plain_conv1(head) and head.stride == (1, 1, 1) and head.out_channels <= 4
+                and head.in_channels == self.out_channels and head.weight.dtype == torch.float32):
+            return False
+        n = x.shape[0] // 2 if planar else x.shape[0]
+        cin = x.shape[1] * 2 if planar else x.shape[1]
+        cout = ops.cpad(self.out_channels) if self._pad else self.out_channels
+        vox = x.shape[2] * x.shape[3] * x.shape[4]
+        return (cin, cout) in ((64, 32), (128, 64)) and n * vox >= 65536 and vox % 16 == 0
+
+    def forward(self, x, in_link=None, out_link=None, planar=False, head=None):
         if self._native and x.is_cuda:
             skip_w = self.skip_conv.weight if self.uses_skip_conv else None
             skip_b = self.skip_conv.bias if self.uses_skip_conv else None
+            head_w = head.weight if head is not None else None
+            head_b = head.bias if head is not None else None
             return ops.ResBlockFn.apply(x, self.conv1.weight, self.conv1.bias, self.conv2.weight, self.conv2.bias,
                                         skip_w, skip_b, self.stride, self._drop_scale(x, planar),
                                         self._in_segs if self._pad else 0,
-                                        self._checkpoint and torch.is_grad_enabled(), in_link, out_link, planar)
+                                        self._checkpoint and torch.is_grad_enabled(), in_link, out_link, planar,
+                                        head_w, head_b)
+        if head is not None:
+            raise N.Ru3dError("ResBlock: a head rides only in the native block (ask takes_head first)")
         if self._native:
             N.require_device(x, "ResBlock input")
         if self._bn_eval and x.is_cuda and _inference_mode(self):
@@ -628,18 +649,26 @@
         x = self.encode_blocks[-1](x)
         levels = self._supervised_levels()
         aux = {}
+        headed = False
         for i in reversed(range(self.num_pool)):
             x = self.up_blocks[i](x, skips[i], links[i]) if linked else self.up_blocks[i](x, skips[i])
-            if linked and getattr(links[i], "planar_out", False):
-                x = self.decode_blocks[i](x, planar=True)
+            planar = bool(linked and getattr(links[i], "planar_out", False))
+            blk = self.decode_blocks[i]
+            headed = (i == 0 and self._in_chain and self._native_io and isinstance(blk, ResBlock)
+                      and not getattr(self.up_blocks[i], "attention", False) and blk.takes_head(x, self.fc, planar))
+            if headed:
+                x = blk(x, planar=planar, head=self.fc)
+            elif planar:
+                x = blk(x, planar=True)
             else:
-                x = self.decode_blocks[i](x)
+                x = blk(x)
             if 1 <= i < levels:
                 aux[i] = self._aux_head(i, x)
         ops._DROP_POOL.clear()
+        out = x if headed else self._head(x)
         if levels:
-            return [self._head(x)] + [aux[l] for l in range(1, levels)]
-        return self._head(x)
+            return [out] + [aux[l] for l in range(1, levels)]
+        return out
 
 
 def _stacks_by_level(level):
diff --git a/include/ru3d.h b/include/ru3d.h
--- a/include/ru3d.h
+++ b/include/ru3d.h
@@ -105,6 +105,13 @@
 size_t ru3d_head_bwd_workspace_bytes(const ru3d_tensor* x, int dtype);
 int ru3d_head_bwd(const ru3d_tensor* x, const ru3d_tensor* dlogits, const float* weight, int cin_real, const ru3d_tensor* dx,
                   float* dw, float* db, void* ws, size_t ws_bytes, int dtype, void* stream);
+int ru3d_head_in_bwd_supported(const ru3d_tensor* z, const ru3d_tensor* dlogits, const ru3d_tensor* y,
+                               const ru3d_tensor* gpre, const ru3d_tensor* dy, int dtype);
+size_t ru3d_head_in_bwd_workspace_bytes(const ru3d_tensor* z, int dtype);
+int ru3d_head_in_bwd(const ru3d_tensor* z, const ru3d_tensor* dlogits, const float* weight, int cin_real,
+                     const ru3d_tensor* y, const float* mean, const float* scale, const ru3d_tensor* gpre,
+                     const ru3d_tensor* dy, float* dw, float* db, float* gpre_sum, void* ws, size_t ws_bytes, float slope,
+                     int dtype, void* stream);
 
 int ru3d_convtranspose3d_k3s2p1_fwd(const ru3d_tensor* x, const void* w_packed, const float* bias,
                                     const ru3d_tensor* y, int dtype, void* stream);
@@ -125,6 +132,11 @@
 int ru3d_skip1x1_in_lrelu_fwd(const ru3d_tensor* x, const void* w_packed, const float* bias, const ru3d_tensor* y,
                               const float* mean, const float* scale, const ru3d_tensor* out, float slope, int dtype,
                               void* stream);
+int ru3d_skip1x1_in_lrelu_head_fwd_supported(const ru3d_tensor* x, const ru3d_tensor* y, const ru3d_tensor* out,
+                                             const ru3d_tensor* logits, int dtype);
+int ru3d_skip1x1_in_lrelu_head_fwd(const ru3d_tensor* x, const void* w_packed, const float* bias, const ru3d_tensor* y,
+                                   const float* mean, const float* scale, const ru3d_tensor* out, const void* head_w_packed,
+                                   const float* head_bias, const ru3d_tensor* logits, float slope, int dtype, void* stream);
 int ru3d_in_lrelu_fwd(const ru3d_tensor* y, const float* mean, const float* scale, const ru3d_tensor* res,
                       const ru3d_tensor* out, float slope, int dtype, void* stream);
 int ru3d_in_lrelu_bwd(const ru3d_tensor* gout, const ru3d_tensor* out, const ru3d_tensor* y, const float* mean,
```

Measured after the change: 276.9 million voxels/s, median of 6. 1.01x the previous value.
